# abiswas-odu/Disco

Hardware: AMD Instinct MI355X
Metric: overlaps/sec (BuildGraph stage), 150 bp reads (higher is better)
Workload: dtype u64; 1 GPU; 50000000 x 150 bp synthetic reads, 30x of 50 x 5000000 bp uniform-random contigs, both strands, error-free, min-overlap 40 (k=39), transitive reduction on, seed 42; reads=50000000, read_len=150, min_overlap=40, parallelism=1 GPU, e_pre=903537181, e_out=45314794, n_contained=4685156, cap_bind_sites=0, asymmetric_pairs=0, probes=5550000000, kmer_hits=2220071992

## Files before the change

disco_amd/csrc/disco_hip.hip:

```cpp
#include <hip/hip_runtime.h>
#include <rocprofiler-sdk-roctx/roctx.h>

#include <algorithm>
#include <atomic>
#include <chrono>
#include <cstdarg>
#include <cstdio>
#include <cstdlib>
#include <cstring>
#include <functional>
#include <fcntl.h>
#include <sys/mman.h>
#include <sys/stat.h>
#include <unistd.h>
#include <string>
#include <memory>
#include <thread>
#include <map>
#include <mutex>
#include <queue>
#include <vector>

#include "../../include/disco_hip.h"
#include "../../include/disco_hip_test.h"
// ... 796 lines not shown
{
    CHK(ensure(c, c->reads_own, words));
    c->d_reads = c->reads_own;
    CHK(ensure(c, c->len_own, n_len));
    c->d_len = c->len_own;
    return DISCO_OK;
}

static u32 extra_cap(const disco_ctx *c) { return (u32)std::min<u64>(std::min(c->d_extra_node.cap, c->d_extra_key.cap), 0xFFFFFFFFull); }

static int grow_big_lists(disco_ctx *c, u64 need) { return ensure_group(c, need, need, c->d_big_list, c->d_big_cnt); }

static bool own_order_wanted(const disco_ctx *c, u64 nq, int *bits)
{
    const u64 order_min = getenv("DISCO_ORDER_MIN_READS") ? (u64)atoll(getenv("DISCO_ORDER_MIN_READS")) : 4096;
    int b = 16;
    while (b < 27 && (1ull << b) < nq) ++b;
    if (const char *e = getenv("DISCO_ORDER_BITS")) b = std::min(std::max(atoi(e), 12), 26);
    *bits = b;
    return !c->order_external && !getenv("DISCO_NO_ORDER") && nq >= order_min && nq > 0;
}

struct IndexCountPlan {
    u64 lo = 0, hi = 0;
    int lpr = 0, nf = 0;
    u32 *ocnt = nullptr, *oslot = nullptr;
    u64 *oitem = nullptr;
    u32 oidbits = 0;
    u32 oshift = 0;
    u32 osub = 0;
    const u64 *list = nullptr;
};

static bool runs_nf_built(int nf, int m) { return (nf == 7 || nf == 12 || nf == 17 || nf == 22 || nf == 27) && m == RUNS_M; }

static int runs_lpr_for(const disco_ctx *c, int nf, u32 max_len, u64 nloc)
{
    int lpr = 0;
    const int m = view(c).m;
    const bool nf_built = runs_nf_built(nf, m);
    const bool nf_generic = nf >= 2 && nf <= 64 && m > 16 && m <= 31 && !getenv("DISCO_NO_GENERIC_RUNS");
    if ((nf_built || nf_generic) && max_len > (u32)c->ks && !getenv("DISCO_NO_RUNS")) {
        const u32 maxwin = max_len - (u32)c->ks;
        const u32 expect = 2u * maxwin / (u32)(nf + 1);
        lpr = maxwin <= 256 ? (maxwin <= 128 && expect <= 20 ? 16 : (expect <= 44 ? 32 : 0)) : 0;
        const double max_gb = getenv("DISCO_RUNS_MAX_GB") ? atof(getenv("DISCO_RUNS_MAX_GB")) : 16.0;
        if ((double)nloc * lpr * 4.0 > max_gb * 1e9) lpr = 0;
    }
    return lpr;
}

static bool two_class_ok(const disco_ctx *c, int S, u64 n, u64 n_long, u32 short_max, bool will_own = false)
{
    if (((c->comm || c->dist_reads) && !c->dist_two_class) || !(c->reads_owned || will_own) || c->prm.max_substitutions || getenv("DISCO_NO_TWO_CLASS")) return false;
    if (S <= VERIFY_SW || n_long == 0 || n_long * (u64)env_int("DISCO_TWO_CLASS_ONE_IN", 5) > n || n + n_long >= (1ull << 31)) return false;
    return runs_lpr_for(c, c->ks - view(c).m + 1, short_max, n) != 0;
}

static int two_class_alloc(disco_ctx *c, u64 n_long, int Sx, u32 short_max)
{
    c->n_long = n_long;
    c->S_ext = Sx;
    int rc = ensure(c, c->d_ovf, c->n_alloc);
    if (rc == DISCO_OK) rc = ensure(c, c->d_full, n_long * (u64)Sx);
    if (rc == DISCO_OK) rc = ensure(c, c->d_long_ids, n_long);
    if (rc == DISCO_OK) rc = ensure(c, c->d_lpos, n_long);
    if (rc == DISCO_OK) rc = ensure(c, c->d_lmeta, n_long);
    if (rc == DISCO_OK) rc = ensure(c, c->d_linfo, n_long);
    if (rc == DISCO_OK) rc = ensure(c, c->d_n_list, 1);
    if (rc != DISCO_OK) {
        free_long_class(c);
        return rc;
    }
    c->S = VERIFY_SW;
    c->tailb = short_max <= 160 ? 160 : 256;
    c->two_class = true;
    if (getenv("DISCO_VERBOSE"))
        fprintf(stderr, "[disco] two classes of rows: %llu of %llu reads are longer than 256 bases, the others up to %u: 64-byte rows + %d-word rows for those\n",
                (unsigned long long)n_long, (unsigned long long)c->n, short_max, Sx);
    return DISCO_OK;
}

static bool binned_order_wanted(disco_ctx *c, u64 n, int obits, int *id_bits)
{
    if (getenv("DISCO_NO_BINNED_ORDER") || getenv("DISCO_NO_ORDERED_FILL") || c->two_class || n != c->n || n >= 0xFFFF0000ull) return false;
    const u64 binned_min = getenv("DISCO_BINNED_ORDER_MIN_READS") ? (u64)atoll(getenv("DISCO_BINNED_ORDER_MIN_READS")) : (1ull << 21);
    if (n < binned_min) return false;
    int idb = 1, lenb = 1;
    while ((1ull << idb) < n) ++idb;
    while ((1u << lenb) <= c->max_len) ++lenb;
    if (obits + lenb + idb > 64) return false;
    if (ensure(c, c->d_rec2, n) != DISCO_OK) {
        (void)hipGetLastError();
        c->err.clear();
        return false;
    }
    *id_bits = idb;
    c->order_spare_bits = 64 - (obits + lenb + idb);
    return true;
}

static int index_count_plan(disco_ctx *c, const DiscoView &v, u64 lo, u64 hi, IndexCountPlan *pl, const u64 *list = nullptr)
{
    const u64 nloc = hi - lo;
    *pl = IndexCountPlan();
    pl->lo = lo;
    pl->hi = hi;
    pl->list = list;
    if (!list) c->order_counted = c->order_ready = c->order_items = false;
    int obits = 0;
    if (!list && lo == c->q_lo && hi == c->q_hi && own_order_wanted(c, nloc, &obits) && !getenv("DISCO_NO_ORDER_FUSE")) {
        const u64 order_buckets = 1ull << obits;
        if (lo == 0 && binned_order_wanted(c, nloc, obits, &c->order_id_bits)) {
            pl->oitem = (u64 *)c->d_rec2.p;
            pl->oidbits = (u32)c->order_id_bits;
            c->order_items = true;
        } else {
            CHK(ensure(c, c->d_ocnt, order_buckets + 1));
            CHK(ensure(c, c->d_oslot, nloc));
            HIPCHK(c, hipMemsetAsync(c->d_ocnt, 0, (order_buckets + 1) * sizeof(u32), c->stream));
            pl->ocnt = c->d_ocnt;
            pl->oslot = c->d_oslot;
        }
        pl->oshift = 32u - (u32)obits;
        c->order_counted = true;
        c->order_counted_lo = lo;
        c->order_counted_hi = hi;
        c->order_counted_bits = obits;
    }
    c->runs_lpr = 0;
    c->runs_n = 0;
    c->runs_by_pos = false;
    const int nf = v.ks - v.m + 1;
    const int lpr = c->S == VERIFY_SW ? runs_lpr_for(c, nf, c->max_len, nloc) : 0;
    if (lpr && nloc) {
        CHK(ensure(c, c->d_runs, nloc * (u64)lpr));
        c->runs_lpr = lpr;
        c->runs_lo = lo;
        c->runs_n = nloc;
        c->runs_by_pos = list != nullptr;
        pl->lpr = lpr;
        pl->nf = nf;
    }
    c->order_sub_bits = 0;
    if (pl->oitem && pl->lpr) {
        const int qbits = std::max(0, std::min(c->order_spare_bits, std::min(c->order_sub_limit, ORDER_SUB_MAX)));
        const u32 nmm_max = c->max_len - (u32)v.m + 1u;
        if (qbits) pl->osub = ((u32)qbits << 24) | ((1u << (qbits + 16)) / nmm_max);
        c->order_sub_bits = qbits;
    }
    return DISCO_OK;
}

typedef void (*IndexRunsFn)(DiscoView, u32 *, ulonglong2 *, u32 *, u64, u64, u32 *, u32 *, u32 *, u64 *, u32, u32, u32, const u64 *);
typedef void (*IndexCountFn)(DiscoView, u32 *, ulonglong2 *, u32 *, u64, u64, u32 *, u32 *, u64 *, u32, u32, const u64 *);
struct IndexCountKernel {
    IndexRunsFn runs = nullptr;
    IndexCountFn plain = nullptr;
};
template <bool COUNT, int NF, int NFMAX, bool LONGK>
static IndexCountKernel index_runs_pick(int lpr)
{
    IndexCountKernel k;
    k.runs = lpr == 16 ? index_runs_kernel<COUNT, NF, 1, NFMAX, LONGK> : index_runs_kernel<COUNT, NF, 2, NFMAX, LONGK>;
    return k;
}
template <bool COUNT>
static IndexCountKernel index_count_pick(int nf, int m, int lpr, bool longk, bool long_class)
{
    if (long_class || !lpr) {
        IndexCountKernel k;
        if (long_class) k.plain = longk ? index_count_kernel<COUNT, true, true> : index_count_kernel<COUNT, false, true>;
        else k.plain = longk ? index_count_kernel<COUNT, true> : index_count_kernel<COUNT>;
        return k;
    }
    if (runs_nf_built(nf, m)) switch (nf) {
        case 7: return index_runs_pick<COUNT, 7, 7, false>(lpr);
        case 12: return index_runs_pick<COUNT, 12, 12, false>(lpr);
        case 17: return index_runs_pick<COUNT, 17, 17, false>(lpr);
        case 22: return index_runs_pick<COUNT, 22, 22, false>(lpr);
        default: return index_runs_pick<COUNT, 27, 27, false>(lpr);
        }
    if (longk) return nf <= 48 ? index_runs_pick<COUNT, 0, 48, true>(lpr) : index_runs_pick<COUNT, 0, 64, true>(lpr);
    if (nf <= 8) return index_runs_pick<COUNT, 0, 8, false>(lpr);
    if (nf <= 12) return index_runs_pick<COUNT, 0, 12, false>(lpr);
    if (nf <= 16) return index_runs_pick<COUNT, 0, 16, false>(lpr);
    if (nf <= 24) return index_runs_pick<COUNT, 0, 24, false>(lpr);
    if (nf <= 32) return index_runs_pick<COUNT, 0, 32, false>(lpr);
    if (nf <= 48) return index_runs_pick<COUNT, 0, 48, false>(lpr);
    return index_runs_pick<COUNT, 0, 64, false>(lpr);
}
static IndexCountKernel index_count_pick(bool count, int nf, int m, int lpr, bool longk, bool long_class)
{
    return count ? index_count_pick<true>(nf, m, lpr, longk, long_class) : index_count_pick<false>(nf, m, lpr, longk, long_class);
}

static int index_count_chunk(disco_ctx *c, const DiscoView &v, const IndexCountPlan &pl, bool count, ulonglong2 *rec_base, u64 a, u64 b)
{
    if (b <= a) return DISCO_OK;
    const dim3 grid((unsigned)((b - a + 255) / 256));
    ulonglong2 *rec = rec_base + 2 * (a - pl.lo);
    u32 *oslot = pl.oslot ? pl.oslot + (a - pl.lo) : nullptr;
    u64 *oitem = pl.oitem ? pl.oitem + (a - pl.lo) : nullptr;
    u32 *okey = pl.list ? nullptr : c->d_okey.p;
    const IndexCountKernel k = index_count_pick(count, pl.nf, v.m, pl.lpr, c->ks > 64, false);
    if (k.runs) hipLaunchKernelGGL(k.runs, grid, dim3(256), 0, c->stream, v, c->d_bkt, rec, okey, a, b, c->d_runs + (a - pl.lo) * (u64)pl.lpr, pl.ocnt, oslot, oitem, pl.oidbits, pl.oshift, pl.osub, pl.list);
    else hipLaunchKernelGGL(k.plain, grid, dim3(256), 0, c->stream, v, c->d_bkt, rec, okey, a, b, pl.ocnt, oslot, oitem, pl.oidbits, pl.oshift, pl.list);
    HIPCHK(c, hipGetLastError());
    return DISCO_OK;
}

static int index_count_long(disco_ctx *c, const DiscoView &v, const IndexCountPlan &pl, bool count, ulonglong2 *rec, u32 *oslot, u64 x_lo, u64 x_hi)
{
    const dim3 g((unsigned)((x_hi - x_lo + 255) / 256));
    hipLaunchKernelGGL(index_count_pick(count, 0, v.m, 0, c->ks > 64, true).plain, g, dim3(256), 0, c->stream, v, c->d_bkt, rec, c->d_okey, x_lo, x_hi, pl.ocnt, oslot, (u64 *)nullptr, 0u, pl.oshift,
                       (const u64 *)nullptr);
    HIPCHK(c, hipGetLastError());
    return DISCO_OK;
}

static bool binned_index_wanted(disco_ctx *c, int logT)
{
    if (getenv("DISCO_NO_BINNED_INDEX") || 2 * c->n >= 0xFFFF0000ull) return false;
    if (logT > BINX_SPAN_BITS && ensure(c, c->d_rec2, 2 * c->n) != DISCO_OK) {
        (void)hipGetLastError();
        c->err.clear();
        return false;
    }
    return true;
}

static int size_bucket_table(disco_ctx *c)
{
    u64 T = 1024;
    int logT = 10;
    double tscale = 2.0;
    if (const char *e = getenv("DISCO_BUCKET_SCALE")) tscale = atof(e);
    while ((double)T < tscale * (double)c->n && logT < 32) {
        T <<= 1;
        logT++;
    }
    c->T = T;
    c->bshift = 64 - logT;
    return logT;
}

static int index_begin(disco_ctx *c)
{
    const int logT = size_bucket_table(c);
    const u64 T = c->T;
    CHK(ensure(c, c->d_bkt, T + 1));
    CHK(ensure(c, c->d_ent, 2 * c->n));
    CHK(ensure(c, c->d_rec, 2 * c->n));
    CHK(ensure(c, c->d_okey, c->n));
    c->adj_imported = false;
    c->binned_index = binned_index_wanted(c, logT);
    if (!c->binned_index) HIPCHK(c, hipMemsetAsync(c->d_bkt, 0, (T + 1) * sizeof(u32), c->stream));
    return DISCO_OK;
}

struct BinxPlan {
    int span = 0, levels = 0, bits[3] = {0, 0, 0};
};
static BinxPlan binx_plan(int logT)
{
    BinxPlan b;
    b.span = std::min(logT, BINX_SPAN_BITS);
    const int prefix = logT - b.span;
    b.levels = (prefix + BINX_MAX_BITS - 1) / BINX_MAX_BITS;
    for (int l = 0; l < b.levels; l++) b.bits[l] = prefix / b.levels + (l < prefix % b.levels ? 1 : 0);
    return b;
}

template <typename R>
static int binx_partition(disco_ctx *c, const char *what, int bits, u32 kshift, u32 total, R *src, R *dst, const R **out, const u32 **part)
{
    const BinxPlan bp = binx_plan(bits);
    const u32 n_part = 1u << (bits - bp.span);
    const u32 tiles = (total + BINX_TILE - 1u) / BINX_TILE;
    u64 hist_len = 1;
    for (int l = 0, done = 0; l < bp.levels; done += bp.bits[l], l++) hist_len = std::max<u64>(hist_len, ((u64)tiles + (1ull << done)) * (1ull << bp.bits[l]) + 1);
    const u64 tab = ((u64)n_part + 1 + 63) & ~63ull;
    CHK(ensure(c, c->d_binx, 4 * tab + hist_len));
    u32 *seg[2] = {c->d_binx.p, c->d_binx.p + tab}, *tb[2] = {c->d_binx.p + 2 * tab, c->d_binx.p + 3 * tab}, *hist = c->d_binx.p + 4 * tab;
    if (getenv("DISCO_VERBOSE"))
        fprintf(stderr, "[disco] binned %s: 2^%d buckets, %u partitions of 2^%d, %d level(s) of %d / %d / %d bits\n", what, bits, n_part, bp.span, bp.levels, bp.bits[0], bp.bits[1], bp.bits[2]);
    u32 pseg = 1, pnb = 1;
    int cur = 0, done = 0;
    for (int l = 0; l < bp.levels; l++) {
        const u32 nseg = 1u << done, nb = 1u << bp.bits[l], shift = kshift + (u32)(bits - done - bp.bits[l]);
        const u32 grid = tiles + nseg;
        const u64 hlen = (u64)grid * nb + 1;
        hipLaunchKernelGGL(binx_segs_kernel, dim3(1), dim3(1024), 0, c->stream, l ? (const u32 *)hist : (const u32 *)nullptr, (const u32 *)tb[cur ^ 1], pseg, pnb, total, seg[cur], tb[cur]);
        HIPCHK(c, hipMemsetAsync(hist, 0, hlen * sizeof(u32), c->stream));
        hipLaunchKernelGGL(binx_hist_kernel<R>, dim3(grid), dim3(BINX_BLOCK), 0, c->stream, (const R *)src, (const u32 *)seg[cur], (const u32 *)tb[cur], nseg, shift, nb, hist);
        CHK((scan_exclusive<u32, u32>(c, hist, hlen, hist, false, nullptr)));
        hipLaunchKernelGGL(binx_scatter_kernel<R>, dim3(grid), dim3(BINX_BLOCK), 0, c->stream, (const R *)src, dst, (const u32 *)seg[cur], (const u32 *)tb[cur], nseg, shift, nb, (const u32 *)hist);
        HIPCHK(c, hipGetLastError());
        std::swap(src, dst);
        pseg = nseg;
        pnb = nb;
        done += bp.bits[l];
        cur ^= 1;
    }
    hipLaunchKernelGGL(binx_segs_kernel, dim3(1), dim3(1024), 0, c->stream, bp.levels ? (const u32 *)hist : (const u32 *)nullptr, (const u32 *)tb[cur ^ 1], pseg, pnb, total, seg[cur],
                       (u32 *)nullptr);
    HIPCHK(c, hipGetLastError());
    *out = src;
    *part = seg[cur];
    return DISCO_OK;
}

static int binned_build_index(disco_ctx *c)
{
    const int logT = 64 - c->bshift;
    const u32 total = (u32)(2 * c->n);
    const ulonglong2 *rec;
    const u32 *part;
    CHK(binx_partition(c, "index build", logT, 32u, total, c->d_rec.p, c->d_rec2.p, &rec, &part));
    const int span = std::min(logT, BINX_SPAN_BITS);
    hipLaunchKernelGGL(binx_build_kernel<ulonglong2>, dim3(1u << (logT - span)), dim3(BINX_BUILD_BLOCK), 0, c->stream, rec, part, (u32)span, 32u, 0u, total, c->T, c->d_bkt.p, c->d_ent.p);
    HIPCHK(c, hipGetLastError());
    return DISCO_OK;
}

static int binned_build_order(disco_ctx *c)
{
    const int bits = c->order_counted_bits + c->order_sub_bits;
    const u32 total = (u32)c->n, kshift = 64u - (u32)bits;
    u64 *items = (u64 *)c->d_rec2.p;
    const u64 *rec;
    const u32 *part;
    CHK(binx_partition(c, "grouping", bits, kshift, total, items, items + c->n, &rec, &part));
    const int span = std::min(bits, BINX_SPAN_BITS);
    hipLaunchKernelGGL(binx_build_kernel<u64>, dim3(1u << (bits - span)), dim3(BINX_BUILD_BLOCK), 0, c->stream, rec, part, (u32)span, kshift, (u32)c->order_id_bits, total, (u64)0,
                       (u32 *)nullptr, c->d_order_own.p);
    HIPCHK(c, hipGetLastError());
    return DISCO_OK;
}

static int start_contained_rows(disco_ctx *c, bool grouped)
{
    const u64 nc = c->n_contained;
    if (c->crows_pending && c->crows_n == nc && (!grouped || c->cgrp_pending)) return DISCO_OK;
    const bool have_rows = c->crows_pending && c->crows_n == nc;
    if (!have_rows) c->crows_pending = c->cgrp_pending = false;
    const u64 max_rows = getenv("DISCO_EAGER_ROWS_MAX") ? (u64)atoll(getenv("DISCO_EAGER_ROWS_MAX")) : (16ull << 20);
    if (c->comm || nc == 0 || nc > max_rows || c->n >= (1ull << 31)) return DISCO_OK;
    if (!c->aux_stream) {
        HIPCHK(c, hipStreamCreateWithFlags(&c->aux_stream, hipStreamNonBlocking));
        HIPCHK(c, hipEventCreateWithFlags(&c->ev_crows, hipEventDisableTiming));
        HIPCHK(c, hipMalloc((void **)&c->d_total2, sizeof(u64)));
    }
    CHK(ensure(c, c->d_cpos, c->n + 1));
    CHK(ensure_group(c, nc, nc + nc / 4 + 1024, c->d_crow_id, c->d_crow_key, c->d_crow_len));
    if (nc > c->crows_hcap && c->h_ring && !c->crows_in_ring && (u64)c->ring_half * 2 >= (nc + 1024) * 32) {
        if (c->h_crows) (void)hipHostFree(c->h_crows);
        c->h_crows = c->h_ring;
        c->crows_hcap = (u64)c->ring_half * 2 / 32;
        c->crows_in_ring = true;
    }
    if (nc > c->crows_hcap) {
        if (c->h_crows && !c->crows_in_ring) (void)hipHostFree(c->h_crows);
        c->crows_in_ring = false;
        c->h_crows = nullptr;
        c->crows_hcap = 0;
        const u64 want = nc + nc / 4 + 1024;
        if (hipHostMalloc(&c->h_crows, want * 32) != hipSuccess) {
            c->h_crows = nullptr;
            (void)hipGetLastError();
            return DISCO_OK;
        }
        c->crows_hcap = want;
    }
    if (!have_rows) {
    CHK((scan_exclusive_on<u8, u32>(c, c->aux_stream, c->d_tile2, c->d_total2, c->d_contained, c->n, c->d_cpos, false, nullptr)));
    hipLaunchKernelGGL(contain_rows32_kernel, dim3(flat_grid(c, c->n)), dim3(256), 0, c->aux_stream, c->d_best, c->d_contained, c->d_cpos, c->n, c->d_crow_id, c->d_crow_key);
    HIPCHK(c, hipGetLastError());
    u64 *hkey = (u64 *)c->h_crows;
    u32 *hid = (u32 *)(hkey + c->crows_hcap), *hln = hid + c->crows_hcap;
    hipLaunchKernelGGL(crow_lens_kernel, dim3(flat_grid(c, nc)), dim3(256), 0, c->aux_stream, (const u32 *)c->d_crow_id, (const u64 *)c->d_crow_key, nc, (const u16 *)c->d_len, c->d_crow_len);
    HIPCHK(c, hipGetLastError());
    HIPCHK(c, hipMemcpyAsync(hkey, c->d_crow_key, nc * 8, hipMemcpyDeviceToHost, c->aux_stream));
    HIPCHK(c, hipMemcpyAsync(hid, c->d_crow_id, nc * 4, hipMemcpyDeviceToHost, c->aux_stream));
    HIPCHK(c, hipMemcpyAsync(hln, c->d_crow_len, nc * 4, hipMemcpyDeviceToHost, c->aux_stream));
    HIPCHK(c, hipEventRecord(c->ev_crows, c->aux_stream));
    c->crows_n = nc;
    c->crows_pending = true;
    }
    if (grouped && !c->cgrp_pending) {
        CHK(ensure(c, c->d_cgrp_cur, c->n + 1));
        CHK(ensure_group(c, nc, nc + nc / 4 + 1024, c->d_cgrp_id, c->d_cgrp_key));
        CHK(ensure(c, c->d_cgrp_big, 1));
        HIPCHK(c, hipMemsetAsync(c->d_cpos, 0, (c->n + 1) * sizeof(u32), c->aux_stream));
        HIPCHK(c, hipMemsetAsync(c->d_cgrp_big, 0, sizeof(u64), c->aux_stream));
        hipLaunchKernelGGL(crow_count_kernel, dim3(flat_grid(c, nc)), dim3(256), 0, c->aux_stream, (const u64 *)c->d_crow_key, nc, c->d_cpos);
        CHK((scan_exclusive_on<u32, u32>(c, c->aux_stream, c->d_tile2, c->d_total2, c->d_cpos, c->n + 1, c->d_cgrp_cur, false, nullptr)));
        hipLaunchKernelGGL(crow_place_kernel, dim3(flat_grid(c, nc)), dim3(256), 0, c->aux_stream, (const u32 *)c->d_crow_id, (const u64 *)c->d_crow_key, nc, c->d_cgrp_cur, c->d_cgrp_id,
                           c->d_cgrp_key);
        hipLaunchKernelGGL(crow_sort_groups_kernel, dim3(flat_grid(c, nc)), dim3(256), 0, c->aux_stream, c->d_cgrp_id, c->d_cgrp_key, nc, c->d_cgrp_big);
        HIPCHK(c, hipGetLastError());
        u64 *gkey = (u64 *)((char *)c->h_crows + c->crows_hcap * 16);
        u32 *gid = (u32 *)(gkey + c->crows_hcap), *gln = gid + c->crows_hcap;
        hipLaunchKernelGGL(crow_lens_kernel, dim3(flat_grid(c, nc)), dim3(256), 0, c->aux_stream, (const u32 *)c->d_cgrp_id, (const u64 *)c->d_cgrp_key, nc, (const u16 *)c->d_len, c->d_crow_len);
        HIPCHK(c, hipMemcpyAsync(gkey, c->d_cgrp_key, nc * 8, hipMemcpyDeviceToHost, c->aux_stream));
        HIPCHK(c, hipMemcpyAsync(gid, c->d_cgrp_id, nc * 4, hipMemcpyDeviceToHost, c->aux_stream));
        HIPCHK(c, hipMemcpyAsync(gln, c->d_crow_len, nc * 4, hipMemcpyDeviceToHost, c->aux_stream));
        HIPCHK(c, hipMemcpyAsync(&c->h_cgrp_big, c->d_cgrp_big, sizeof(u64), hipMemcpyDeviceToHost, c->aux_stream));
        c->cgrp_pending = true;
    }
    return DISCO_OK;
}

static int settle_contained_rows(disco_ctx *c)
{
    if (c->crows_pending) HIPCHK(c, hipStreamSynchronize(c->aux_stream));
    c->crows_pending = false;
    c->cgrp_pending = false;
    return DISCO_OK;
}

static int ring_back_from_rows(disco_ctx *c)
{
    if (!c->crows_in_ring) return DISCO_OK;
    if (c->crows_pending && c->aux_stream) HIPCHK(c, hipStreamSynchronize(c->aux_stream));
    c->crows_pending = c->cgrp_pending = false;
    c->h_crows = nullptr;
    c->crows_hcap = 0;
    c->crows_in_ring = false;
    return DISCO_OK;
}

static void settle_hits_prealloc(disco_ctx *c)
{
    if (!c->hits_prealloc.joinable()) return;
    c->hits_prealloc.join();
    c->hbm_bytes -= std::exchange(c->prealloc_asked, 0) * 8;
    if (c->prealloc && c->prealloc.cap > c->d_hits.cap) {
        release(c, c->d_hits);
        adopt(c, c->d_hits, c->prealloc);
    } else if (c->prealloc)
        (void)hipFree(c->prealloc.p);
    c->prealloc = DevBuf<u64>();
}


typedef void (*ProbeFn)(ProbeArgs);
typedef void (*ProbeRunsFn)(ProbeArgs, const u32 *, u64);
struct ProbeKernel {
    ProbeRunsFn runs = nullptr;
    ProbeFn plain = nullptr;
};
template <int PMODE>
static ProbeFn probe_mode_pick(bool ldsrow, bool row17, bool longk, bool long_class)
{
    if constexpr (PMODE != 0) {
        if (long_class) return longk ? probe_kernel<PMODE, false, false, true, true> : row17 ? probe_kernel<PMODE, false, true, false, true> : probe_kernel<PMODE, false, false, false, true>;
    }
    if constexpr (PMODE != 2) {
        if (!ldsrow) return longk ? probe_kernel<PMODE, false, false, true> : row17 ? probe_kernel<PMODE, false, true> : probe_kernel<PMODE, false, false>;
    }
    return longk ? probe_kernel<PMODE, true, false, true> : row17 ? probe_kernel<PMODE, true, true> : probe_kernel<PMODE, true, false>;
}
static ProbeKernel probe_pick(const disco_ctx *c, int mode, bool use_runs)
{
    const bool ldsrow = c->S <= PROBE_ACAP;
    const bool row17 = c->ks - view(c).m == 16 && !getenv("DISCO_NO_ROW17");
    const bool longk = c->ks > 64;
    const bool long_class = c->two_class && c->S_ext > PROBE_ACAP;
    ProbeKernel k;
    if (mode == 0 && use_runs) k.runs = c->k != c->ks ? (c->runs_lpr == 16 ? probe_runs_kernel<16, true> : probe_runs_kernel<32, true>) : (c->runs_lpr == 16 ? probe_runs_kernel<16> : probe_runs_kernel<32>);
    else if (mode == 0) k.plain = probe_mode_pick<0>(ldsrow, row17, longk, long_class);
    else if (mode == 1) k.plain = probe_mode_pick<1>(ldsrow, row17, longk, long_class);
    else k.plain = probe_mode_pick<2>(ldsrow, row17, longk, long_class);
    return k;
}

typedef void (*VerifyFn)(VerifyArgs);
template <bool INEXACT>
static VerifyFn verify_rows_pick(int S, bool short_rows)
{
    if (S == VERIFY_SW) return short_rows ? verify_kernel<5, 0, INEXACT> : verify_kernel<8, 0, INEXACT>;
    return S == 16 ? verify_kernel<16, 0, INEXACT> : S == 24 ? verify_kernel<24, 0, INEXACT> : S == 32 ? verify_kernel<32, 0, INEXACT> : verify_kernel<0, 0, INEXACT>;
}
template <int MODE>
static VerifyFn verify_pass_pick(bool flat, bool short_rows)
{
    if (flat) return short_rows ? verify_flat_kernel<5, MODE> : verify_flat_kernel<8, MODE>;
// ... 341 lines not shown
        return fail(c, DISCO_E_ARG, "%llu reads have a length outside (min_overlap=%u, min(32767, 32*stride)]", (unsigned long long)c->h_ctr[CTR_BAD_LEN], c->prm.min_overlap);
    c->max_len = (u32)c->h_ctr[CTR_MAX_LEN];
    c->phase = 1;
    return DISCO_OK;
}

struct ReadShape {
    u64 n = 0;
    uint32_t stride = 0;
    u64 n_long = 0;
    u32 short_max = 0, longest = 0, shortest = 0;
};

static void set_read_lengths(disco_ctx *c, u32 longest, u32 short_max, u32 shortest)
{
    c->max_len_all = longest;
    c->max_len = c->two_class ? short_max : longest;
    c->min_len = shortest;
}

static void drop_reads(disco_ctx *c) { (void)set_reads_common(c, 0, VERIFY_SW, nullptr); }

static int begin_rows(disco_ctx *c, u64 n, u64 n_alloc, u64 extra_rows, uint32_t stride, bool may_keep, bool spare_hits = false)
{
    LocalBuf<u64> hits(c);
    bool kept = false;
    if (spare_hits) hits.take(c->d_hits);
    const int rc = set_reads_common(c, n, stride, may_keep ? &kept : nullptr);
    if (spare_hits) hits.give(c->d_hits);
    CHK(rc);
    c->reads_owned = true;
    c->n_alloc = n_alloc;
    return kept ? DISCO_OK : alloc_reads(c, (n_alloc + extra_rows) * (u64)stride, n_alloc);
}

static int begin_read_table(disco_ctx *c, const ReadShape &s, bool spare_hits = false)
{
    const bool classes = two_class_ok(c, (int)s.stride, s.n, s.n_long, s.short_max, true);
    CHK(begin_rows(c, s.n, s.n, classes ? s.n_long : 0, classes ? (uint32_t)VERIFY_SW : s.stride, !classes, spare_hits));
    if (classes) CHK(two_class_alloc(c, s.n_long, (int)s.stride, s.short_max));
    set_read_lengths(c, s.longest, s.short_max, s.shortest);
    return DISCO_OK;
}

static int number_long_reads(disco_ctx *c, u32 *ovf, u32 *ids, u64 *count)
{
    hipLaunchKernelGGL(class_flag_kernel, dim3(flat_grid(c, c->n)), dim3(256), 0, c->stream, (const u16 *)c->d_len, c->n, ovf, c->d_ctr);
    CHK((scan_exclusive<u32, u32>(c, ovf, c->n, ovf, false, count)));
    if (ids) hipLaunchKernelGGL(class_ids_kernel, dim3(flat_grid(c, c->n)), dim3(256), 0, c->stream, (const u16 *)c->d_len, (const u32 *)ovf, c->n, ids);
    return DISCO_OK;
}

static int upload_reads_impl(disco_ctx *c, const char *who, const uint64_t *packed, uint32_t stride_words, const uint16_t *len, uint64_t n)
{
    if (!c || (n && (!packed || !len))) return c ? fail(c, DISCO_E_ARG, "%s: null argument", who) : DISCO_E_ARG;
    HIPCHK(c, hipSetDevice(c->device));
    const bool ragged = stride_words == 0;
    const auto t_begin = std::chrono::steady_clock::now();
    auto lapms = [&]() { return std::chrono::duration<double, std::milli>(std::chrono::steady_clock::now() - t_begin).count(); };
    double t_scan = 0, t_alloc = 0, t_issued = 0, t_mirror = 0;
    u64 CH = getenv("DISCO_UPLOAD_CHUNK") ? (u64)atoll(getenv("DISCO_UPLOAD_CHUNK")) : (4ull << 20);
    if (!ragged) CH = std::min<u64>(CH, (512ull << 20) / ((u64)stride_words * 8));
    CH = std::max<u64>((CH + 255) & ~255ull, 256);
    const u64 n_chunks = (n + CH - 1) / CH;
    u64 n_bad = 0;
    ReadShape shape{n, 0, 0, 0, 0, n ? 0xFFFFu : 0u};
    std::vector<u64> chunk_words(n_chunks + 1, 0);
    {
        const u32 mo = c->prm.min_overlap, cap = ragged ? 32767u : std::min<u32>(32767u, stride_words * 32u);
        std::mutex mu;
        parallel_for(n, [&](u64 b0, u64 e0) {
            u64 bad = 0, nlong = 0;
            u32 mx = 0, mn = 0xFFFFu, smx = 0;
            for (u64 k = b0 / CH; k * CH < e0; k++) {
                u64 words = 0;
                for (u64 i = std::max<u64>(b0, k * CH); i < std::min<u64>(e0, (k + 1) * CH); i++) {
                    const u32 L = len[i];
                    bad += (L <= mo || L > cap);
                    mx = std::max(mx, L);
                    mn = std::min(mn, L);
                    nlong += L > (u32)DISCO_SHORT_MAX;
                    if (L <= (u32)DISCO_SHORT_MAX) smx = std::max(smx, L);
                    words += (L + 31u) >> 5;
                }
                std::lock_guard<std::mutex> lk(mu);
                chunk_words[k + 1] += words;
            }
            std::lock_guard<std::mutex> lk(mu);
            n_bad += bad;
            shape.n_long += nlong;
            shape.longest = std::max(shape.longest, mx);
            shape.shortest = std::min(shape.shortest, mn);
            shape.short_max = std::max(shape.short_max, smx);
        });
        for (u64 k = 0; k < n_chunks; k++) chunk_words[k + 1] += chunk_words[k];
    }
    if (ragged) stride_words = std::max<u32>(1, (shape.longest + 31) / 32);
    t_scan = lapms();
    const uint32_t dstride = shape.stride = (stride_words + 7u) & ~7u;
    if (n_bad) {
        drop_reads(c);
        return fail(c, DISCO_E_ARG, "%llu reads have a length outside (min_overlap=%u, min(32767, 32*stride)]", (unsigned long long)n_bad, c->prm.min_overlap);
    }
    CHK(begin_read_table(c, shape));
    const bool classes = c->two_class;
    if (n) {
        CHK(ensure_copy_stream(c));
        CHK(copy_stream_after_stream(c));
        const bool direct = !ragged && !classes && dstride == stride_words;
        const bool eager = !c->comm && !classes && !getenv("DISCO_NO_EAGER_INDEX");
        HIPCHK(c, hipMemcpyAsync(c->d_len, len, n * 2, hipMemcpyHostToDevice, c->stream));
        u64 ring_words = 0;
        for (u64 k = 0; k < n_chunks; k++)
            ring_words = std::max<u64>(ring_words, ragged ? chunk_words[k + 1] - chunk_words[k] : (std::min<u64>(n, (k + 1) * CH) - k * CH) * (u64)stride_words);
        if (!direct) CHK(ensure(c, c->d_dense, 3 * ring_words));
        LocalBuf<u64> woff(c);
        LocalBuf<u32> nw(c);
        if (ragged) {
            CHK(ensure(c, woff, n));
            CHK(ensure(c, nw, n));
            hipLaunchKernelGGL(words_per_read_kernel, dim3(flat_grid(c, n)), dim3(256), 0, c->stream, (const u16 *)c->d_len, n, nw);
            CHK((scan_exclusive<u32, u64>(c, nw, n, woff, false, nullptr)));
        }
        if (classes) CHK(number_long_reads(c, c->d_ovf, c->d_long_ids, nullptr));
        t_alloc = lapms();
        IndexCountPlan pl;
        DiscoView v;
        if (eager) {
            CHK(index_begin(c));
            v = view(c);
            CHK(index_count_plan(c, v, 0, n, &pl));
        }
        for (u64 k = 0; k < n_chunks; k++) {
            const u64 lo = k * CH, hi = std::min<u64>(n, lo + CH);
            const int b = (int)(k % 3);
            if (!direct) {
                u64 *ring = c->d_dense + (u64)b * ring_words;
                const u64 w0 = ragged ? chunk_words[k] : lo * (u64)stride_words, w1 = ragged ? chunk_words[k + 1] : hi * (u64)stride_words;
                if (k >= 3) HIPCHK(c, hipStreamWaitEvent(c->copy_stream, c->ev_unpacked[b], 0));
                HIPCHK(c, hipMemcpyAsync(ring, packed + w0, (w1 - w0) * 8, hipMemcpyHostToDevice, c->copy_stream));
                HIPCHK(c, hipEventRecord(c->ev_copied[b], c->copy_stream));
                HIPCHK(c, hipStreamWaitEvent(c->stream, c->ev_copied[b], 0));
                hipLaunchKernelGGL(unpack_reads_kernel, dim3(flat_grid(c, (hi - lo) * (u64)c->S)), dim3(256), 0, c->stream, (const u64 *)ring, ragged ? 0 : (int)stride_words, (const u64 *)woff, w0,
                                   (const u16 *)c->d_len, lo, hi, c->S, classes ? (u32)DISCO_SHORT_MAX : 0xFFFFu, c->d_reads);
                if (classes)
                    hipLaunchKernelGGL(unpack_long_reads_kernel, dim3(flat_grid(c, shape.n_long * ((u64)dstride + 8))), dim3(256), 0, c->stream, (const u64 *)ring, ragged ? 0 : (int)stride_words,
                                       (const u64 *)woff, w0, (const u16 *)c->d_len, lo, hi, (const u32 *)c->d_long_ids, shape.n_long, n, (int)dstride, c->tailb, c->d_full, c->d_reads);
                HIPCHK(c, hipEventRecord(c->ev_unpacked[b], c->stream));
            } else {
                HIPCHK(c, hipMemcpyAsync(c->d_reads + lo * dstride, packed + lo * dstride, (hi - lo) * (u64)dstride * 8, hipMemcpyHostToDevice, c->copy_stream));
                HIPCHK(c, hipEventRecord(c->ev_copied[b], c->copy_stream));
                HIPCHK(c, hipStreamWaitEvent(c->stream, c->ev_copied[b], 0));
            }
            if (eager) CHK(index_count_chunk(c, v, pl, !c->binned_index, c->d_rec, lo, hi));
        }
        HIPCHK(c, hipGetLastError());
        t_issued = lapms();
        if (c->h_len.size() != n) c->h_len.resize(n);
        uint16_t *hl = c->h_len.data();
        parallel_for(n, [&, hl](u64 b0, u64 e0) { memcpy(hl + b0, len + b0, (e0 - b0) * 2); });
        c->h_len_ok = true;
        t_mirror = lapms();
        HIPCHK(c, hipStreamSynchronize(c->copy_stream));
        if (getenv("DISCO_VERBOSE"))
            fprintf(stderr, "[disco] %s: lengths checked %.1f ms, buffers %.1f, chunks issued %.1f, lengths mirrored %.1f, copies done %.1f (%s%s)\n", who, t_scan, t_alloc, t_issued,
                    t_mirror, lapms(), classes ? "two classes of rows" : "one stride", eager ? ", index counted behind the copies" : "");
        if (woff) HIPCHK(c, hipStreamSynchronize(c->stream));
        c->index_counted = eager;
    } else
        c->h_len.clear();
    c->phase = 1;
    return DISCO_OK;
}

int disco_upload_reads(disco_ctx *c, const uint64_t *packed, uint32_t stride_words, const uint16_t *len, uint64_t n)
{
    DISCO_TRACE("disco_upload_reads");
    if (c && stride_words == 0) return fail(c, DISCO_E_ARG, "stride_words 0 out of range");
    return upload_reads_impl(c, "disco_upload_reads", packed, stride_words, len, n);
}

int disco_upload_reads_ragged(disco_ctx *c, const uint64_t *words, const uint16_t *len, uint64_t n)
{
    DISCO_TRACE("disco_upload_reads_ragged");
    return upload_reads_impl(c, "disco_upload_reads_ragged", words, 0, len, n);
}

namespace {
enum { DP_STARTS = 0, DP_GOOD, DP_TOO_LONG, DP_MAX_LEN, DP_MIN_LEN_INV, DP_N_LONG, DP_SHORT_MAX, DP_COUNT };

struct IngestPiece {
    u64 p0 = 0, p1 = 0;
    u64 own_lo = 0, own_hi = 0, n = 0;
    bool to_eof = false;
    bool prefix_nl = true, last_nl = false;
    u64 own_nl = 0, tiles = 0;
    u8 *d_text = nullptr;
    u64 *d_tile_base = nullptr, *d_ctr = nullptr;
    u32 *d_tile_cnt = nullptr;
    u64 *d_start = nullptr, *d_seq = nullptr;
    u32 *d_wrap = nullptr;
    u16 *d_glen = nullptr;
    u64 n_start = 0, good = 0;
    u64 fig[DP_COUNT] = {0, 0, 0, 0, 0, 0, 0};
};

struct IngestFile {
    std::string path;
    int fd = -1;
    char last = 0;
    bool fastq = false;
    u64 n = 0;
    const u8 *map = nullptr;
    u64 comp_n = 0;
    u8 *d_comp = nullptr;
    std::vector<infl::BgzfBlock> blocks;
    uint64_t m_first = 0, m_count = 0;
    IngestPiece p;
};
}

static void ingest_tables(FxTables *tb)
{
    memset(tb, 0, sizeof *tb);
    auto code = [](char ch) { return ch == 'A' ? 0ull : (ch == 'C' ? 1ull : (ch == 'G' ? 2ull : 3ull)); };
    tb->n_rep = (u32)DISCO_N_END_REPEATS;
    for (u32 r = 0; r < tb->n_rep; r++) {
        u64 v = 0;
        for (int x = 0; x < 29; x++) v = (v << 2) | code(kEndRepeats[r][x]);
        tb->rep58[r] = v;
    }
    tb->n_motif = (u32)DISCO_N_MOTIFS;
    for (u32 m = 0; m < tb->n_motif; m++) {
        const size_t l = strlen(kMotifs[m]);
        tb->motif_len[m] = (u8)l;
        for (size_t x = 0; x < l; x++) {
            tb->motif[m][x] = (u8)kMotifs[m][x];
            tb->need[m][code(kMotifs[m][x])]++;
        }
    }
    static_assert(DISCO_N_END_REPEATS <= FX_MAX_REPEATS && DISCO_N_MOTIFS <= FX_MAX_MOTIFS, "filter tables");
}

static unsigned ring_alloc_flags()
{
    const int mode = env_int("DISCO_RING_MODE", 0);
    return mode == 1 ? hipHostMallocNonCoherent : (mode == 2 ? hipHostMallocCoherent : hipHostMallocDefault);
}

static const size_t RING_HALF = 128u << 20;
static int pinned_ring(disco_ctx *c, const char *who)
{
    CHK(ring_back_from_rows(c));
    if (!c->h_ring) {
        if (hipHostMalloc(&c->h_ring, 2 * RING_HALF, ring_alloc_flags()) != hipSuccess) {
            c->h_ring = nullptr;
            (void)hipGetLastError();
            return fail(c, DISCO_E_NOMEM, "%s: no pinned staging memory", who);
        }
        c->ring_half = RING_HALF;
        for (int i = 0; i < 2; i++) HIPCHK(c, hipEventCreateWithFlags(&c->ev_ring[i], hipEventDisableTiming));
    }
    return DISCO_OK;
}
static int ingest_ring(disco_ctx *c)
{
    CHK(pinned_ring(c, "disco_ingest_fasta"));
    return ensure_copy_stream(c);
}

static int ingest_read_file(disco_ctx *c, int fd, u64 n, u8 *d_text, unsigned threads, u64 file_off = 0, void *own_ring = nullptr, size_t own_ring_bytes = 0)
{
    constexpr unsigned RING_SLOTS = 4;
    const size_t HALF = 128u << 20, SLOT = own_ring ? own_ring_bytes / RING_SLOTS : 2 * HALF / RING_SLOTS;
    if (own_ring) CHK(ensure_copy_stream(c));
    else CHK(ingest_ring(c));
    char *const h_ring = own_ring ? (char *)own_ring : (char *)c->h_ring;
    hipEvent_t ev[RING_SLOTS] = {own_ring ? c->ev_copied[2] : c->ev_ring[0], own_ring ? c->ev_unpacked[1] : c->ev_ring[1], c->ev_copied[0], c->ev_copied[1]};
    threads = (unsigned)env_int("DISCO_INGEST_THREADS", (int)std::min(threads, 6u));
    threads = std::max(1u, std::min(threads, 64u));
    CHK(copy_stream_after_stream(c));
    const u64 n_chunks = (n + SLOT - 1) / SLOT;
    const u64 n_pieces = n_chunks * threads;
    std::atomic<u64> next_piece{0};
    std::vector<std::atomic<int>> slot_free(n_chunks), pieces_in(n_chunks);
    for (u64 k = 0; k < n_chunks; k++) {
        slot_free[k].store(k < RING_SLOTS ? 1 : 0);
        pieces_in[k].store(0);
    }
    std::atomic<bool> ok{true}, stop{false};
    auto nap = [] { std::this_thread::sleep_for(std::chrono::microseconds(30)); };
    std::vector<std::thread> th;
    for (unsigned t = 0; t < threads; t++)
        th.emplace_back([&]() {
            for (;;) {
                const u64 p = next_piece.fetch_add(1);
                if (p >= n_pieces) return;
                const u64 k = p / threads;
                const unsigned piece = (unsigned)(p % threads);
                while (!slot_free[k].load(std::memory_order_acquire)) {
                    if (stop.load()) return;
                    nap();
                }
                const u64 off = k * (u64)SLOT;
                const size_t len = (size_t)std::min<u64>(SLOT, n - off);
                char *slot = h_ring + (k % RING_SLOTS) * SLOT;
                size_t p0 = len * piece / threads, p1 = len * (piece + 1) / threads;
// ... 610 lines not shown
            });
    }
    return DISCO_OK;
}

extern "C" int disco_ingest_fetch(disco_ctx *c, uint16_t *len, uint64_t *file_index)
{
    if (!c || !len || !file_index) return c ? fail(c, DISCO_E_ARG, "disco_ingest_fetch: null argument") : DISCO_E_ARG;
    if (c->phase < 1 || c->ingest_n == 0 || c->ingest_n != c->n) return fail(c, DISCO_E_STATE, "disco_ingest_fetch: the reads of the context did not come from disco_ingest_fasta");
    HIPCHK(c, hipSetDevice(c->device));
    const u64 n = c->n;
    CHK(ingest_fetch_range(c, 0, n, c->copy_stream ? c->copy_stream : c->stream, len, file_index));
    {
        std::lock_guard<std::mutex> lk(c->h_len_mu);
        if (!(c->h_len_ok && c->h_len.size() == n)) {
            if (c->h_len.size() != n) c->h_len.resize(n);
            uint16_t *hl = c->h_len.data();
            parallel_for(n, [&, hl](u64 b, u64 e_) { memcpy(hl + b, len + b, (e_ - b) * 2); });
            c->h_len_ok = true;
        }
    }
    return DISCO_OK;
}

int disco_adopt_reads(disco_ctx *c, const void *d_packed, uint32_t stride_words, const void *d_len, uint64_t n)
{
    if (!c || (n && (!d_packed || !d_len))) return c ? fail(c, DISCO_E_ARG, "disco_adopt_reads: null argument") : DISCO_E_ARG;
    HIPCHK(c, hipSetDevice(c->device));
    CHK(set_reads_common(c, n, stride_words));
    c->d_reads = (u64 *)d_packed;
    c->d_len = (u16 *)d_len;
    c->reads_owned = false;
    return validate_reads(c);
}

static int gen_spec(disco_ctx *c, const char *who, const disco_genspec_abi *s, disco_genspec *g, uint32_t *stride)
{
    memcpy(g, s, sizeof *g);
    const uint32_t longest = std::max<uint32_t>(s->len_max, DISCO_GEN_LONG_SHARE(g) ? DISCO_GEN_LONG_LEN(g) : 0u);
    if (s->len_min == 0 || s->len_max < s->len_min || longest > 32767 || s->n_contigs == 0 || s->contig_len < longest) return fail(c, DISCO_E_ARG, "%s: bad spec", who);
    *stride = (((longest + 31) / 32) + 7u) & ~7u;
    return DISCO_OK;
}

int disco_generate_reads(disco_ctx *c, const disco_genspec_abi *s)
{
    DISCO_TRACE("disco_generate_reads");
    if (!c || !s) return c ? fail(c, DISCO_E_ARG, "disco_generate_reads: null argument") : DISCO_E_ARG;
    disco_genspec g;
    ReadShape shape;
    CHK(gen_spec(c, "disco_generate_reads", s, &g, &shape.stride));
    HIPCHK(c, hipSetDevice(c->device));
    shape.n = s->n_reads;
    CHK(begin_read_table(c, shape));
    if (c->n) hipLaunchKernelGGL(generate_reads_kernel, dim3(flat_grid(c, c->n * shape.stride)), dim3(256), 0, c->stream, g, c->d_reads, c->d_len, (int)shape.stride, (u64)0, c->n);
    HIPCHK(c, hipGetLastError());
    return validate_reads(c);
}

int disco_substitute_bases(disco_ctx *c, uint64_t seed, uint32_t rate_ppm)
{
    if (!c) return DISCO_E_ARG;
    if (c->phase != 1) return fail(c, DISCO_E_STATE, "disco_substitute_bases: call after the reads are set and before disco_build_index");
    if (rate_ppm > 1000000) return fail(c, DISCO_E_ARG, "disco_substitute_bases: rate above 10^6 ppm");
    if (c->two_class)
        return fail(c, DISCO_E_UNSUPPORTED, "disco_substitute_bases: the table has two classes of rows (reads of more than 256 bases next to short ones); substitute "
                                            "into generated reads, or set DISCO_NO_TWO_CLASS=1");
    HIPCHK(c, hipSetDevice(c->device));
    const u64 lo = c->comm ? c->q_lo : 0, hi = c->comm ? c->q_hi : c->n;
    if (hi > lo && rate_ppm)
        hipLaunchKernelGGL(substitute_bases_kernel, dim3(flat_grid(c, (hi - lo) * (u64)c->S)), dim3(256), 0, c->stream, (u64)seed, rate_ppm, c->d_reads, c->d_len, c->S, lo, hi);
    c->index_counted = c->order_counted = c->order_ready = false;
    HIPCHK(c, hipGetLastError());
    return DISCO_OK;
}

int disco_download_reads(disco_ctx *c, uint64_t *packed, uint16_t *len)
{
    if (!c || c->phase < 1) return c ? fail(c, DISCO_E_STATE, "no reads") : DISCO_E_ARG;
    HIPCHK(c, hipSetDevice(c->device));
    LocalBuf<u64> joined(c);
    if (packed && c->n && c->two_class) {
        CHK(ensure(c, joined, c->n * (u64)c->S_ext));
        hipLaunchKernelGGL(class_join_kernel, dim3(flat_grid(c, c->n * (u64)c->S_ext)), dim3(256), 0, c->stream, (const u64 *)c->d_reads, (const u64 *)c->d_full, c->S_ext,
                           (const u16 *)c->d_len, (const u32 *)c->d_ovf, c->n, joined);
        (void)hipMemcpyAsync(packed, joined, c->n * (u64)c->S_ext * 8, hipMemcpyDeviceToHost, c->stream);
    } else if (packed && c->n)
        HIPCHK(c, hipMemcpyAsync(packed, c->d_reads, c->n * (u64)c->S * 8, hipMemcpyDeviceToHost, c->stream));
    if (len && c->n) (void)hipMemcpyAsync(len, c->d_len, c->n * 2, hipMemcpyDeviceToHost, c->stream);
    const hipError_t e = hipStreamSynchronize(c->stream);
    if (e != hipSuccess) return fail(c, DISCO_E_HIP, "disco_download_reads: %s", hipGetErrorString(e));
    return DISCO_OK;
}

uint32_t disco_stride_words(const disco_ctx *c) { return c ? (uint32_t)(c->two_class ? c->S_ext : c->S) : 0; }
uint64_t disco_num_reads(const disco_ctx *c) { return c ? c->n : 0; }
uint64_t disco_long_rows(const disco_ctx *c) { return c && c->two_class ? c->n_long : 0; }

int disco_set_query_range(disco_ctx *c, uint64_t lo, uint64_t hi)
{
    if (!c) return DISCO_E_ARG;
    if (c->phase < 1 || c->phase > 2) return fail(c, DISCO_E_STATE, "disco_set_query_range: call after the reads are set and before disco_probe");
    if (lo > hi || hi > c->n) return fail(c, DISCO_E_ARG, "query range [%llu,%llu) outside [0,%llu)", (unsigned long long)lo, (unsigned long long)hi, (unsigned long long)c->n);
    c->q_lo = lo;
    c->q_hi = hi;
    return DISCO_OK;
}

static int two_class_convert(disco_ctx *c)
{
    if (c->two_class || !c->n || c->max_len <= (u32)DISCO_SHORT_MAX || !two_class_ok(c, c->S, c->n, 1, (u32)c->k + 1)) return DISCO_OK;
    const int Sx = c->S;
    LocalBuf<u32> ovf(c);
    CHK(ensure(c, ovf, c->n_alloc));
    CHK(zero_counter(c, CTR_SHORT_MAX));
    u64 n_long = 0;
    CHK(number_long_reads(c, ovf, nullptr, &n_long));
    CHK(read_counters(c));
    const u32 short_max = (u32)c->h_ctr[CTR_SHORT_MAX];
    if (!two_class_ok(c, Sx, c->n, n_long, short_max)) return DISCO_OK;
    LocalBuf<u64> rows8(c);
    ovf.give(c->d_ovf);
    int rca = ensure(c, rows8, (c->n + n_long) * 8);
    if (rca == DISCO_OK) rca = two_class_alloc(c, n_long, Sx, short_max);
    if (rca != DISCO_OK) {
        free_long_class(c);
        return rca;
    }
    hipLaunchKernelGGL(class_split_kernel, dim3(flat_grid(c, c->n * 8)), dim3(256), 0, c->stream, (const u64 *)c->reads_own, Sx, (const u16 *)c->d_len, (const u32 *)c->d_ovf, c->n, c->tailb,
                       rows8.p, c->d_full, c->d_long_ids);
    HIPCHK(c, hipGetLastError());
    HIPCHK(c, hipStreamSynchronize(c->stream));
    rows8.give(c->reads_own);
    c->d_reads = c->reads_own;
    set_read_lengths(c, c->max_len, short_max, c->min_len);
    return DISCO_OK;
}

int disco_build_index(disco_ctx *c)
{
    DISCO_TRACE("disco_build_index");
    if (!c) return DISCO_E_ARG;
    if (c->phase < 1) return fail(c, DISCO_E_STATE, "disco_build_index: no reads");
    HIPCHK(c, hipSetDevice(c->device));
    ph_begin(c, DISCO_PH_INDEX);
    if (c->index_counted) {
        c->index_counted = false;
    } else {
        CHK(two_class_convert(c));
        CHK(index_begin(c));
        const DiscoView v = view(c);
        IndexCountPlan pl;
        CHK(index_count_plan(c, v, 0, c->n, &pl));
        CHK(index_count_chunk(c, v, pl, !c->binned_index, c->d_rec, 0, c->n));
        if (c->two_class) CHK(index_count_long(c, v, pl, !c->binned_index, c->d_rec, pl.oslot, 0, c->n_long));
    }
    const bool binned = c->binned_index;
    if (!binned) CHK((scan_exclusive<u32, u32>(c, c->d_bkt, c->T + 1, c->d_bkt, false, nullptr)));
    c->order_ready = false;
    if (c->order_counted && c->order_counted_lo == 0 && c->order_counted_hi == c->n && !c->two_class && !getenv("DISCO_NO_ORDERED_FILL")) {
        const u64 order_buckets = 1ull << c->order_counted_bits;
        CHK(ensure(c, c->d_order_own, c->n));
        ph_end(c, DISCO_PH_INDEX);
        ph_begin(c, DISCO_PH_ORDER);
        if (c->order_items) CHK(binned_build_order(c));
        else {
            CHK((scan_exclusive<u32, u32>(c, c->d_ocnt, order_buckets + 1, c->d_ocnt, false, nullptr)));
            hipLaunchKernelGGL(order_scatter_kernel, dim3(flat_grid(c, c->n)), dim3(256), 0, c->stream, c->d_okey, c->d_oslot, c->d_ocnt, 32u - (u32)c->order_counted_bits, (u64)0, c->n, c->d_len, c->d_order_own);
        }
        ph_end(c, DISCO_PH_ORDER);
        ph_begin(c, DISCO_PH_INDEX2);
        if (binned) CHK(binned_build_index(c));
        else hipLaunchKernelGGL(index_fill_ordered_kernel, dim3(flat_grid(c, c->n)), dim3(256), 0, c->stream, c->n, (const u64 *)c->d_order_own, (const ulonglong2 *)c->d_rec, (const u32 *)c->d_bkt, c->d_ent);
        ph_end(c, DISCO_PH_INDEX2);
        HIPCHK(c, hipGetLastError());
        c->order_ready = true;
        c->phase = 2;
        return DISCO_OK;
    }
    if (binned) CHK(binned_build_index(c));
    else if (c->n) hipLaunchKernelGGL(index_fill_kernel, dim3(flat_grid(c, 2 * c->n)), dim3(256), 0, c->stream, 2 * c->n, c->d_rec, c->d_bkt, c->d_ent);
    HIPCHK(c, hipGetLastError());
    ph_end(c, DISCO_PH_INDEX);
    c->phase = 2;
    return DISCO_OK;
}

int disco_probe(disco_ctx *c)
{
    DISCO_TRACE("disco_probe");
    if (!c) return DISCO_E_ARG;
    if (c->phase < 2) return fail(c, DISCO_E_STATE, "disco_probe: build the index first");
    HIPCHK(c, hipSetDevice(c->device));
    CHK(settle_contained_rows(c));
    CHK(settle_keys(c));
    drop_edge_records(c);
    drop_contained_records(c);
    settle_hits_prealloc(c);
    const u64 nq = c->q_hi - c->q_lo;
    CHK(ensure(c, c->d_best, c->n_alloc));
    CHK(ensure(c, c->d_row_start, c->n));
    CHK(ensure(c, c->d_row_cnt, c->n));
    if (c->n_alloc) hipLaunchKernelGGL(fill_u64_kernel, dim3(flat_grid(c, c->n_alloc)), dim3(256), 0, c->stream, c->d_best, c->n_alloc, DISCO_NOKEY);
    HIPCHK(c, hipMemsetAsync(c->d_row_cnt, 0, std::max<u64>(c->n, 1) * sizeof(u32), c->stream));
    const bool use_runs = c->runs_lpr != 0 && c->d_runs && c->q_lo >= c->runs_lo && c->q_hi <= c->runs_lo + c->runs_n;
    const ProbeKernel range_kernel = probe_pick(c, 0, use_runs);
    const int grid = range_kernel.runs ? wq_grid(c, range_kernel.runs, nq, "DISCO_PROBE_WAVES") : wq_grid(c, range_kernel.plain, nq, "DISCO_PROBE_WAVES");
    auto launch_probe = [&](const ProbeArgs &a, const ProbeKernel &k, int g) {
        if (k.runs) hipLaunchKernelGGL(k.runs, dim3(g), dim3(64), 0, c->stream, a, (const u32 *)c->d_runs, c->runs_by_pos ? ~0ull : c->runs_lo);
        else hipLaunchKernelGGL(k.plain, dim3(g), dim3(64), 0, c->stream, a);
    };
    const u64 chunk_slots = use_runs ? PR_CHUNK : PROBE_CHUNK;
    u64 want_hits = nq * 64 + (u64)grid * chunk_slots + (1u << 16);
    u32 want_slow = use_runs ? (u32)std::min<u64>(nq, nq / 64 + 1024 + (c->two_class ? c->n_long : 0)) : 1u;
    u32 want_big = (u32)std::min<u64>(nq, nq / 64 + 1024);
    for (int attempt = 0; attempt < 8; attempt++) {
        if (want_hits > c->d_hits.cap) {
            release(c, c->d_hits);
            size_t fr = 0, tot = 0;
            HIPCHK(c, hipMemGetInfo(&fr, &tot));
            if (want_hits * 8 > fr) {
                u64 can = fr / 8 / 10 * 9;
                if (can < (u64)grid * chunk_slots * 2) return fail(c, DISCO_E_NOMEM, "disco_probe: not enough HBM for the hit buffer (%llu entries wanted)", (unsigned long long)want_hits);
                want_hits = can;
            }
            CHK(ensure(c, c->d_hits, want_hits));
        }
        if (want_slow > c->d_slow_list.cap) CHK(ensure(c, c->d_slow_list, want_slow));
        CHK(grow_big_lists(c, want_big));
        HIPCHK(c, hipMemsetAsync(c->d_bump, 0, sizeof(u64), c->stream));
        HIPCHK(c, hipMemsetAsync(c->d_n_big, 0, sizeof(u32), c->stream));
        HIPCHK(c, hipMemsetAsync(c->d_n_slow, 0, sizeof(u32), c->stream));
        HIPCHK(c, hipMemsetAsync(c->d_ctr + CTR_KMER_HITS, 0, sizeof(u64) * 4, c->stream));
        CHK(zero_counter(c, CTR_MAX_ROW));
        CHK(zero_counter(c, CTR_ES_BIG));
        CHK(zero_counter(c, CTR_ES_MID));
        c->es_big_counted = c->tr_big_counted = false;
        ProbeArgs a;
        a.v = view(c);
        a.hits = c->d_hits;
        a.row_start = c->d_row_start;
        a.row_cnt = c->d_row_cnt;
        c->h_probe_rare.bump = c->d_bump;
        c->h_probe_rare.hits_cap = c->d_hits.cap;
        c->h_probe_rare.big_list = c->d_big_list;
        c->h_probe_rare.big_cnt = c->d_big_cnt;
        c->h_probe_rare.n_big = c->d_n_big;
        c->h_probe_rare.big_cap = c->d_big_list.cap;
        c->h_probe_rare.slow_cap = c->d_slow_list.cap;
        c->h_probe_rare.slow_list = c->d_slow_list;
        c->h_probe_rare.n_slow = c->d_n_slow;
        c->h_probe_rare.ctr = c->d_ctr;
        CHK(ensure(c, c->d_probe_rare, 1));
        HIPCHK(c, hipMemcpyAsync(c->d_probe_rare, &c->h_probe_rare, sizeof(ProbeRare), hipMemcpyHostToDevice, c->stream));
        a.rare = c->d_probe_rare;
        CHK(ensure(c, c->d_meta_ord, std::max<u64>(nq, 1)));
        a.meta_ord = c->d_meta_ord;
        int order_bits = 16;
        const bool own_order = own_order_wanted(c, nq, &order_bits);
        a.order = nullptr;
        const u64 order_buckets = 1ull << order_bits;
        const bool counted = c->order_counted && c->order_counted_lo == c->q_lo && c->order_counted_hi == c->q_hi && c->order_counted_bits == order_bits &&
                             (!c->order_items || c->order_ready);
        c->order_counted = false;
        if (c->loci) {
            c->d_order_used = c->d_order_own;
        } else if (own_order && c->order_ready && counted) {
            c->d_order_used = c->d_order_own;
        } else if (own_order) {
            CHK(ensure(c, c->d_ocnt, order_buckets + 1));
            CHK(ensure(c, c->d_oslot, nq));
            CHK(ensure(c, c->d_order_own, nq));
            const u32 oshift = 32u - (u32)order_bits;
            ph_begin(c, DISCO_PH_ORDER);
            if (!counted) {
                HIPCHK(c, hipMemsetAsync(c->d_ocnt, 0, (order_buckets + 1) * sizeof(u32), c->stream));
                hipLaunchKernelGGL(order_count_kernel, dim3(flat_grid(c, nq)), dim3(256), 0, c->stream, c->d_okey + c->q_lo, nq, oshift, c->d_ocnt, c->d_oslot);
            }
            CHK((scan_exclusive<u32, u32>(c, c->d_ocnt, order_buckets + 1, c->d_ocnt, false, nullptr)));
            hipLaunchKernelGGL(order_scatter_kernel, dim3(flat_grid(c, nq)), dim3(256), 0, c->stream, c->d_okey + c->q_lo, c->d_oslot, c->d_ocnt, oshift, c->q_lo, nq, c->d_len, c->d_order_own);
            ph_end(c, DISCO_PH_ORDER);
            HIPCHK(c, hipGetLastError());
            c->d_order_used = c->d_order_own;
        } else if (c->order_external && nq) {
            CHK(ensure(c, c->d_order_own, nq));
            hipLaunchKernelGGL(order_pack_kernel, dim3(flat_grid(c, nq)), dim3(256), 0, c->stream, c->d_order, nq, c->d_len, c->d_order_own);
            HIPCHK(c, hipGetLastError());
            c->d_order_used = c->d_order_own;
        } else
            c->d_order_used = nullptr;
        a.order = c->d_order_used;
        c->order_q_lo = c->q_lo;
        c->order_q_hi = c->q_hi;
        ph_begin(c, DISCO_PH_PROBE_KERNEL);
        HIPCHK(c, hipMemsetAsync(c->d_wq, 0, sizeof(u64) * WQ_WORDS, c->stream));
        const bool partitioned = c->dist_active && c->part_index;
        if (partitioned) CHK(dist_partitioned_probe(c));
        else if (nq) {
            launch_probe(a, range_kernel, grid);
        }
        ph_end(c, DISCO_PH_PROBE_KERNEL);
        HIPCHK(c, hipGetLastError());
        u32 n_big = 0, n_slow = 0;
        if (!partitioned) {
            HIPCHK(c, hipMemcpyAsync(&n_slow, c->d_n_slow, sizeof(u32), hipMemcpyDeviceToHost, c->stream));
            HIPCHK(c, hipMemcpyAsync(&n_big, c->d_n_big, sizeof(u32), hipMemcpyDeviceToHost, c->stream));
        }
        CHK(read_counters(c));
// ... 2404 lines not shown
        sc[(size_t)p] = scnt[(size_t)p] * elem;
        a += sc[(size_t)p];
        ro[(size_t)p] = b;
        rc[(size_t)p] = rcnt[(size_t)p] * elem;
        b += rc[(size_t)p];
        if (p != c->comm->rank) c->dinfo.bytes_sent[xid] += sc[(size_t)p];
    }
    const auto t0 = HClock::now();
    COMM_CHK(c, c->comm->all_to_all_v(send, so.data(), sc.data(), recv, ro.data(), rc.data(), c->stream));
    if (c->time_exchanges) HIPCHK(c, hipStreamSynchronize(c->stream));
    c->dinfo.ms[xid] += ms_since(t0);
    return DISCO_OK;
}

static u64 vsum(const std::vector<u64> &v)
{
    u64 s = 0;
    for (u64 x : v) s += x;
    return s;
}

static int host_reduce(disco_ctx *c, u64 *vals, int n, bool take_max = false)
{
    const int G = c->comm->world;
    std::vector<u64> all((size_t)G * n);
    COMM_CHK(c, c->comm->host_all_gather((const unsigned long long *)vals, n, (unsigned long long *)all.data(), c->stream));
    for (int i = 0; i < n; i++) {
        u64 a = 0;
        for (int p = 0; p < G; p++) a = take_max ? std::max(a, all[(size_t)p * n + i]) : a + all[(size_t)p * n + i];
        vals[i] = a;
    }
    return DISCO_OK;
}

template <int W>
static int dist_deal_rows(disco_ctx *c)
{
    typedef ReadItem<W> Item;
    const u64 nhome = c->home_hi - c->home_lo;
    const u64 per16 = (sizeof(Item) + 15) / 16;
    CHK(ensure(c, c->d_x16a, std::max<u64>(2 * nhome * per16, 1)));
    Item *items = (Item *)c->d_x16a.p, *sorted = (Item *)(c->d_x16a + nhome * per16);
    if (nhome) hipLaunchKernelGGL(read_items_kernel<W>, dim3(flat_grid(c, nhome * (W + 1))), dim3(256), 0, c->stream, (const u64 *)c->d_reads, (const u16 *)c->d_len, c->S, c->home_lo, c->home_hi, items);
    HIPCHK(c, hipGetLastError());
    std::vector<u64> scnt, rcnt;
    RouteByReadItem<W> f{c->d_otab};
    CHK(route_items(c, items, nhome, f, sorted, scnt));
    CHK(exchange_counts(c, scnt, rcnt));
    const u64 nr = vsum(rcnt);
    if (nr != c->n_own) return fail(c, DISCO_E_STATE, "dealt reads: %llu rows arrive for %llu own reads", (unsigned long long)nr, (unsigned long long)c->n_own);
    CHK(ensure(c, c->d_x16b, std::max<u64>(nr * per16, 1)));
    CHK(a2a_items(c, DISCO_X_READS_DEALT, sorted, scnt, c->d_x16b, rcnt, sizeof(Item)));
    if (nr) hipLaunchKernelGGL(read_items_place_kernel<W>, dim3(flat_grid(c, nr * (W + 1))), dim3(256), 0, c->stream, (const Item *)c->d_x16b.p, nr, c->S, c->d_reads, c->d_len);
    HIPCHK(c, hipGetLastError());
    return DISCO_OK;
}

static int dist_deal_reads(disco_ctx *c)
{
    DISCO_TRACE("dist_deal_reads");
    const u32 G = (u32)c->comm->world, r = (u32)c->comm->rank;
    const u64 hlo = c->home_lo, hhi = c->home_hi;
    CHK(ensure(c, c->d_okey, c->n_alloc));
    CHK(ensure(c, c->d_otab, c->n_alloc));
    DiscoView v = view(c);
    if (hhi > hlo) {
        if (v.m == RUNS_M) hipLaunchKernelGGL(read_keys_kernel<true>, dim3((unsigned)((hhi - hlo + 255) / 256)), dim3(256), 0, c->stream, v, hlo, hhi, c->d_okey);
        else hipLaunchKernelGGL(read_keys_kernel<false>, dim3((unsigned)((hhi - hlo + 255) / 256)), dim3(256), 0, c->stream, v, hlo, hhi, c->d_okey);
    }
    HIPCHK(c, hipGetLastError());
    {
        const auto t0 = HClock::now();
        COMM_CHK(c, c->comm->all_gather(c->d_okey + (u64)r * c->per, c->d_okey, c->per * sizeof(u32), c->stream));
        c->dinfo.bytes_sent[DISCO_X_KEYS] += (u64)(G - 1) * c->per * sizeof(u32);
        c->dinfo.ms[DISCO_X_KEYS] += ms_since(t0);
    }
    CHK(ensure(c, c->d_own_ids, std::max<u64>(c->n, 1)));
    CHK(ensure(c, c->d_list_n, 1));
    HIPCHK(c, hipMemsetAsync(c->d_list_n, 0, sizeof(u64), c->stream));
    int obits = 16;
    const bool order_own = own_order_wanted(c, std::max<u64>(c->n / G, 1), &obits) && !getenv("DISCO_DIST_ORDER_TWO_PASSES");
    const u32 oshift = 32u - (u32)obits;
    if (order_own) {
        CHK(ensure(c, c->d_ocnt, (1ull << obits) + 1));
        CHK(ensure(c, c->d_oslot, std::max<u64>(c->n, 1)));
        HIPCHK(c, hipMemsetAsync(c->d_ocnt, 0, ((1ull << obits) + 1) * sizeof(u32), c->stream));
    }
    if (c->n) hipLaunchKernelGGL(own_select_kernel, dim3((unsigned)std::min<u64>((c->n + OWN_TILE - 1) / OWN_TILE, (u64)c->n_cu * 16)), dim3(256), 0, c->stream, (const u32 *)c->d_okey, c->n, G, r,
                                 c->d_otab, c->d_own_ids, c->d_list_n, order_own ? c->d_ocnt : (u32 *)nullptr, order_own ? c->d_oslot : (u32 *)nullptr, oshift);
    HIPCHK(c, hipGetLastError());
    u64 n_own = 0;
    HIPCHK(c, hipMemcpyAsync(&n_own, c->d_list_n, sizeof(u64), hipMemcpyDeviceToHost, c->stream));
    HIPCHK(c, counted_stream_sync(c->stream));
    c->n_own = n_own;
    c->loci = true;
    c->q_lo = 0;
    c->q_hi = n_own;
    if (c->wait_bulk_before_verify) {
        const int W = (int)((c->max_len + 31) / 32);
        if (W <= 5 && c->S >= 5 && !getenv("DISCO_DIST_NO_DEAL_ROWS")) CHK(dist_deal_rows<5>(c));
        else if (W <= 8 && c->S >= 8 && !getenv("DISCO_DIST_NO_DEAL_ROWS")) CHK(dist_deal_rows<8>(c));
        else {
            HIPCHK(c, hipStreamWaitEvent(c->stream, c->ev_bulk, 0));
            c->wait_bulk_before_verify = false;
        }
    }
    CHK(ensure(c, c->d_order_own, std::max<u64>(n_own, 1)));
    ph_begin(c, DISCO_PH_ORDER);
    int obits2 = 16;
    const bool order_two = !order_own && own_order_wanted(c, n_own, &obits2);
    if ((order_own && n_own) || order_two) {
        const int ob = order_own ? obits : obits2;
        const u64 order_buckets = 1ull << ob;
        const u32 oshift = 32u - (u32)ob;
        if (order_two) {
            CHK(ensure(c, c->d_ocnt, order_buckets + 1));
            CHK(ensure(c, c->d_oslot, n_own));
            HIPCHK(c, hipMemsetAsync(c->d_ocnt, 0, (order_buckets + 1) * sizeof(u32), c->stream));
            hipLaunchKernelGGL(order_count_list_kernel, dim3(flat_grid(c, n_own)), dim3(256), 0, c->stream, (const u32 *)c->d_okey, (const u32 *)c->d_own_ids, n_own, G, r, oshift, c->d_ocnt, c->d_oslot);
        }
        CHK((scan_exclusive<u32, u32>(c, c->d_ocnt, order_buckets + 1, c->d_ocnt, false, nullptr)));
        hipLaunchKernelGGL(order_scatter_list_kernel, dim3(flat_grid(c, n_own)), dim3(256), 0, c->stream, (const u32 *)c->d_okey, (const u32 *)c->d_own_ids, (const u32 *)c->d_oslot,
                           (const u32 *)c->d_ocnt, n_own, G, r, oshift, (const u16 *)c->d_len, c->d_order_own);
    } else if (n_own)
        hipLaunchKernelGGL(order_pack_list_kernel, dim3(flat_grid(c, n_own)), dim3(256), 0, c->stream, (const u32 *)c->d_own_ids, n_own, (const u16 *)c->d_len, c->d_order_own);
    ph_end(c, DISCO_PH_ORDER);
    HIPCHK(c, hipGetLastError());
    c->d_order_used = c->d_order_own;
    c->order_counted = false;
    c->dinfo.own_reads = n_own;
    return DISCO_OK;
}

static int dist_build_index(disco_ctx *c)
{
    DISCO_TRACE("dist_build_index");
    const u32 G = (u32)c->comm->world, r = (u32)c->comm->rank;
    const u64 nloc = c->q_hi - c->q_lo;
    const int logT = size_bucket_table(c);
    const u64 T = c->T;
    auto blo_of = [&](u64 g) { return (g * T + G - 1) / G; };
    const u64 blo = blo_of(r), bhi = blo_of(r + 1);
    const bool part = c->part_index;
    if (!part) {
        CHK(ensure(c, c->d_bkt, T + 1));
        CHK(ensure(c, c->d_ent, 2 * c->n));
    }
    CHK(ensure(c, c->d_okey, c->loci ? c->n_alloc : c->n));
    CHK(ensure(c, c->d_rec, std::max<u64>(2 * nloc, 1)));
    c->adj_imported = false;
    ph_begin(c, DISCO_PH_INDEX);
    DiscoView v = view(c);
    IndexCountPlan pl;
    if (c->loci) {
        CHK(index_count_plan(c, v, 0, c->n_own, &pl, c->d_order_own));
        CHK(index_count_chunk(c, v, pl, false, c->d_rec, 0, c->n_own));
    } else {
        CHK(index_count_plan(c, v, c->q_lo, c->q_hi, &pl));
        CHK(index_count_chunk(c, v, pl, false, c->d_rec, c->q_lo, c->q_hi));
        if (c->two_class && nloc) {
            u32 xb[2] = {0, (u32)c->n_long};
            HIPCHK(c, hipMemcpyAsync(&xb[0], c->d_ovf + c->q_lo, sizeof(u32), hipMemcpyDeviceToHost, c->stream));
            if (c->q_hi < c->n) HIPCHK(c, hipMemcpyAsync(&xb[1], c->d_ovf + c->q_hi, sizeof(u32), hipMemcpyDeviceToHost, c->stream));
            HIPCHK(c, hipStreamSynchronize(c->stream));
            if (xb[1] > xb[0]) {
                ulonglong2 *rec_by_id = c->d_rec - 2 * (ptrdiff_t)c->q_lo;
                u32 *oslot_by_id = pl.oslot ? pl.oslot - (ptrdiff_t)c->q_lo : nullptr;
                CHK(index_count_long(c, v, pl, false, rec_by_id, oslot_by_id, xb[0], xb[1]));
            }
        }
    }
    CHK(ensure(c, c->d_x16a, std::max<u64>(2 * nloc, 1)));
    std::vector<u64> scnt, rcnt, matrix;
    RouteByBucket f{logT, G};
    CHK(route_items(c, c->d_rec.p, 2 * nloc, f, c->d_x16a.p, scnt));
    CHK(exchange_counts(c, scnt, rcnt, &matrix));
    const u64 nrec = vsum(rcnt);
    CHK(ensure(c, c->d_x16b, std::max<u64>(nrec, 1)));
    CHK(a2a_items(c, DISCO_X_INDEX_RECORDS, c->d_x16a, scnt, c->d_x16b, rcnt, sizeof(ulonglong2)));
    std::vector<u64> shard((size_t)G, 0);
    for (u32 p = 0; p < G; p++)
        for (u32 q = 0; q < G; q++) shard[q] += matrix[(size_t)p * G + q];
    u64 base = 0;
    for (u32 q = 0; q < r; q++) base += shard[q];
    if (shard[r] != nrec) return fail(c, DISCO_E_STATE, "index shard: %llu records received, %llu announced", (unsigned long long)nrec, (unsigned long long)shard[r]);
    if (vsum(shard) != 2 * c->n) return fail(c, DISCO_E_STATE, "index: %llu records over all ranks, expected %llu", (unsigned long long)vsum(shard), (unsigned long long)(2 * c->n));
    if (part) {
        CHK(ensure(c, c->d_bkt, bhi - blo + 1));
        CHK(ensure(c, c->d_ent, std::max<u64>(nrec, 1)));
        u32 *bkt0 = c->d_bkt - blo;
        HIPCHK(c, hipMemsetAsync(c->d_bkt, 0, (bhi - blo + 1) * sizeof(u32), c->stream));
        if (nrec) hipLaunchKernelGGL(shard_count_kernel, dim3(flat_grid(c, nrec)), dim3(256), 0, c->stream, c->d_x16b, nrec, bkt0);
        CHK((scan_exclusive<u32, u32>(c, c->d_bkt, bhi - blo + 1, c->d_bkt, false, nullptr)));
        if (nrec) hipLaunchKernelGGL(index_fill_kernel, dim3(flat_grid(c, nrec)), dim3(256), 0, c->stream, nrec, c->d_x16b, bkt0, c->d_ent);
        HIPCHK(c, hipGetLastError());
        c->part_blo = blo;
        c->part_bhi = bhi;
        c->part_nrec = nrec;
        ph_end(c, DISCO_PH_INDEX);
        c->phase = 2;
        return DISCO_OK;
    }
    if (bhi > blo) HIPCHK(c, hipMemsetAsync(c->d_bkt + blo, 0, (bhi - blo) * sizeof(u32), c->stream));
    if (nrec) hipLaunchKernelGGL(shard_count_kernel, dim3(flat_grid(c, nrec)), dim3(256), 0, c->stream, c->d_x16b, nrec, c->d_bkt);
    if (bhi > blo) {
        CHK((scan_exclusive<u32, u32>(c, c->d_bkt + blo, bhi - blo, c->d_bkt + blo, false, nullptr)));
        if (base) hipLaunchKernelGGL(add_u32_kernel, dim3(flat_grid(c, bhi - blo)), dim3(256), 0, c->stream, c->d_bkt + blo, bhi - blo, (u32)base);
    }
    if (nrec) hipLaunchKernelGGL(index_fill_kernel, dim3(flat_grid(c, nrec)), dim3(256), 0, c->stream, nrec, c->d_x16b, c->d_bkt, c->d_ent);
    const u32 total = (u32)(2 * c->n);
    HIPCHK(c, hipMemcpyAsync(c->d_bkt + T, &total, sizeof(u32), hipMemcpyHostToDevice, c->stream));
    HIPCHK(c, hipGetLastError());
    HIPCHK(c, hipStreamSynchronize(c->stream));
    {
        std::vector<size_t> off((size_t)G), cnt((size_t)G);
        const auto t0 = HClock::now();
        for (u32 p = 0; p < G; p++) {
            off[p] = blo_of(p) * sizeof(u32);
            cnt[p] = (blo_of(p + 1) - blo_of(p)) * sizeof(u32);
        }
        c->dinfo.bytes_sent[DISCO_X_INDEX_SHARDS] += (u64)(G - 1) * cnt[r];
        COMM_CHK(c, c->comm->all_gather_v(c->d_bkt + blo, c->d_bkt, off.data(), cnt.data(), c->stream));
        size_t a = 0;
        for (u32 p = 0; p < G; p++) {
            off[p] = a;
            cnt[p] = shard[p] * sizeof(u64);
            a += cnt[p];
        }
        c->dinfo.bytes_sent[DISCO_X_INDEX_SHARDS] += (u64)(G - 1) * cnt[r];
        COMM_CHK(c, c->comm->all_gather_v(c->d_ent + base, c->d_ent, off.data(), cnt.data(), c->stream));
        HIPCHK(c, hipStreamSynchronize(c->stream));
        c->dinfo.ms[DISCO_X_INDEX_SHARDS] += ms_since(t0);
    }
    ph_end(c, DISCO_PH_INDEX);
    c->phase = 2;
    return DISCO_OK;
}

static int dist_partitioned_probe(disco_ctx *c)
{
    DISCO_TRACE("dist_partitioned_probe");
    const u32 G = (u32)c->comm->world, r = (u32)c->comm->rank;
    const u64 lo = c->q_lo, nloc = c->q_hi - c->q_lo;
    DiscoView v = view(c);
    const int nf = v.ks - v.m + 1;
    const bool seeded = c->k != c->ks;
    const bool have_runs = c->runs_lpr != 0 && c->runs_lo == lo && c->runs_n == nloc;
    int logT = 0;
    while ((1ull << logT) < c->T) ++logT;
    CHK(ensure(c, c->d_list_n, 1));
    u32 *d_nslow = c->d_n_slow;
    auto make = [&](ulonglong2 *out, bool collect_slow) {
        const int grid = flat_grid(c, nloc * (u64)c->runs_lpr);
        u32 *slow = collect_slow ? (u32 *)c->d_slow_list.p : nullptr;
        const u32 cap = c->d_slow_list.cap * 2;
        auto fn = seeded ? (c->runs_lpr == 16 ? pq_make_kernel<16, true> : pq_make_kernel<32, true>) : (c->runs_lpr == 16 ? pq_make_kernel<16> : pq_make_kernel<32>);
        hipLaunchKernelGGL(fn, dim3(grid), dim3(256), 0, c->stream, v, (const u32 *)c->d_runs, lo, c->q_hi, r, out, c->d_list_n, slow, cap, d_nslow);
    };
    u64 nq_fast = 0, n_slow = 0;
    const u32 *slow = nullptr;
    if (have_runs) {
        u32 ns = 0;
        for (int attempt = 0;; attempt++) {
            const u32 want = attempt ? ns / 2 + 1024 : (u32)std::min<u64>(nloc, nloc / 128 + 1024);
            if (want > c->d_slow_list.cap) CHK(ensure(c, c->d_slow_list, want));
            HIPCHK(c, hipMemsetAsync(c->d_list_n, 0, sizeof(u64), c->stream));
            HIPCHK(c, hipMemsetAsync(d_nslow, 0, sizeof(u32), c->stream));
            if (nloc) make(nullptr, true);
            HIPCHK(c, hipGetLastError());
            HIPCHK(c, hipMemcpyAsync(&nq_fast, c->d_list_n, sizeof(u64), hipMemcpyDeviceToHost, c->stream));
            HIPCHK(c, hipMemcpyAsync(&ns, d_nslow, sizeof(u32), hipMemcpyDeviceToHost, c->stream));
            HIPCHK(c, hipStreamSynchronize(c->stream));
            if (ns <= c->d_slow_list.cap * 2 || attempt) break;
        }
        if (ns > c->d_slow_list.cap * 2) return fail(c, DISCO_E_CAPACITY, "dist_partitioned_probe: slow list could not be sized");
        n_slow = ns;
        slow = (const u32 *)c->d_slow_list.p;
    } else
        n_slow = nloc;
    u64 nq_slow = 0, nqs = 0;
    {
    LocalBuf<u32> slow_cnt(c);
    LocalBuf<u64> slow_start(c);
    if (n_slow) {
        CHK(ensure(c, slow_cnt, n_slow));
        CHK(ensure(c, slow_start, n_slow + 1));
        if (seeded) hipLaunchKernelGGL((pq_slow_kernel<true, true>), dim3(flat_grid(c, n_slow, 64)), dim3(64), 0, c->stream, v, slow, n_slow, lo, r, slow_cnt, (const u64 *)nullptr, (ulonglong2 *)nullptr);
        else if (c->ks > 64) hipLaunchKernelGGL(pq_slow_kernel<true>, dim3(flat_grid(c, n_slow, 64)), dim3(64), 0, c->stream, v, slow, n_slow, lo, r, slow_cnt, (const u64 *)nullptr, (ulonglong2 *)nullptr);
        else hipLaunchKernelGGL(pq_slow_kernel<false>, dim3(flat_grid(c, n_slow, 64)), dim3(64), 0, c->stream, v, slow, n_slow, lo, r, slow_cnt, (const u64 *)nullptr, (ulonglong2 *)nullptr);
        CHK((scan_exclusive<u32, u64>(c, slow_cnt, n_slow, slow_start, false, &nq_slow)));
    }
    nqs = nq_fast + nq_slow;
    CHK(ensure(c, c->d_x16a, std::max<u64>(2 * nqs, 1)));
    HIPCHK(c, hipMemsetAsync(c->d_list_n, 0, sizeof(u64), c->stream));
    if (have_runs && nloc) make(c->d_x16a, false);
    if (n_slow) {
        if (seeded) hipLaunchKernelGGL((pq_slow_kernel<true, true>), dim3(flat_grid(c, n_slow, 64)), dim3(64), 0, c->stream, v, slow, n_slow, lo, r, slow_cnt, (const u64 *)slow_start, c->d_x16a + nq_fast);
        else if (c->ks > 64) hipLaunchKernelGGL(pq_slow_kernel<true>, dim3(flat_grid(c, n_slow, 64)), dim3(64), 0, c->stream, v, slow, n_slow, lo, r, slow_cnt, (const u64 *)slow_start, c->d_x16a + nq_fast);
        else hipLaunchKernelGGL(pq_slow_kernel<false>, dim3(flat_grid(c, n_slow, 64)), dim3(64), 0, c->stream, v, slow, n_slow, lo, r, slow_cnt, (const u64 *)slow_start, c->d_x16a + nq_fast);
    }
    if (hipGetLastError() != hipSuccess || hipStreamSynchronize(c->stream) != hipSuccess) return fail(c, DISCO_E_HIP, "dist_partitioned_probe: query kernels failed");
    }
    c->slow_rows = have_runs ? n_slow : 0;
    std::vector<u64> scnt, rcnt;
    RouteByBucket fb{logT, G};
    ulonglong2 *q_sorted = c->d_x16a + nqs;
    CHK(route_items(c, c->d_x16a.p, nqs, fb, q_sorted, scnt));
    CHK(exchange_counts(c, scnt, rcnt));
    const u64 nq_in = vsum(rcnt);
    CHK(ensure(c, c->d_x16b, std::max<u64>(nq_in, 1)));
    CHK(a2a_items(c, DISCO_X_QUERIES, q_sorted, scnt, c->d_x16b, rcnt, sizeof(ulonglong2)));
    CHK(ensure(c, c->d_deg_tmp, std::max<u64>(nq_in, 1)));
    CHK(ensure(c, c->d_pq_start, nq_in + 1));
    const u32 *bkt = c->d_bkt;
    u64 n_hits_out = 0;
    auto answer_count = seeded ? pq_answer_kernel<false, true> : pq_answer_kernel<false, false>;
    auto answer_fill = seeded ? pq_answer_kernel<true, true> : pq_answer_kernel<true, false>;
    if (nq_in) hipLaunchKernelGGL(answer_count, dim3(flat_grid(c, nq_in)), dim3(256), 0, c->stream, (const ulonglong2 *)c->d_x16b, nq_in, bkt, (const u64 *)c->d_ent, c->part_blo, c->per,
                                  nf, c->k - c->ks, c->d_deg_tmp, (const u64 *)nullptr, (ulonglong2 *)nullptr);
    CHK((scan_exclusive<u32, u64>(c, c->d_deg_tmp, nq_in, c->d_pq_start, false, &n_hits_out)));
    CHK(ensure_keep(c, c->d_x16a, std::max<u64>(2 * n_hits_out, 1), 0));
// ... 1420 lines not shown
```

disco_amd/csrc/disco_kernels.h:

```cpp
#ifndef DISCO_KERNELS_H_
#define DISCO_KERNELS_H_

#include "disco_device.h"
#include "readgen.h"

#define PROBE_ROWCAP 512
#define PROBE_SEGW 128
#define PROBE_SEGP (PROBE_SEGW + 64)
#define PROBE_ACAP 32
#define PROBE_CHUNK 4096
#define ES_MID 1024
#define ES_DUPBITS 11
#define ES_DUPTAB (1 << ES_DUPBITS)
#ifndef ES_CAP
#define ES_CAP 256
#endif
#ifndef TR_CAP
#define TR_CAP 256
#endif
#define TR_CAP_SMALL 128
#define VERIFY_SW 8
#define ORDER_BUCKET(key, shift) (((key) * 0x9E3779B1u) >> (shift))
#define SCAN_ITEMS 16
#define SCAN_BLOCK 256
// ... 65 lines not shown
template <u32 CHUNK = WQ_CHUNK>
__device__ __forceinline__ bool wq_grab(u64 *counter, u64 n, u64 &beg, u64 &end)
{
    u64 b = 0;
    if ((threadIdx.x & 63) == 0) b = atomicAdd(counter, (u64)CHUNK);
#ifdef WQ_EXP_SHFL
    b = __shfl(b, 0);
#else
    b = uniform_u64(b);
#endif
    beg = b;
    end = (b + CHUNK < n) ? b + CHUNK : n;
    return b < n;
}

template <u32 CHUNK = WQ_CHUNK, u32 MULT = 4>
__device__ __forceinline__ bool wq_grab_multi(u64 *counter, u64 n, u64 &beg, u64 &end, u64 &gnext, u64 &gend)
{
    if (gnext >= gend) {
        if (!wq_grab<CHUNK * MULT>(counter, n, gnext, gend)) return false;
    }
    beg = gnext;
    end = beg + CHUNK < gend ? beg + CHUNK : gend;
    gnext = end;
    return true;
}

#define WQ_NQ 8u
#define WQ_WORDS (16u * WQ_NQ)
struct WqSplit {
    u32 qi = 0;
};
template <u32 CHUNK = WQ_CHUNK>
__device__ __forceinline__ bool wq_grab_split(u64 *counters, u64 n, u64 &beg, u64 &end, WqSplit &st)
{
    const u32 nchunks = (u32)((n + CHUNK - 1u) / CHUNK);
    const u32 per = (nchunks + WQ_NQ - 1u) / WQ_NQ;
    while (st.qi < WQ_NQ) {
        const u32 q = ((u32)blockIdx.x + st.qi) % WQ_NQ;
        const u32 first = q * per;
        const u32 mine = first < nchunks ? (nchunks - first < per ? nchunks - first : per) : 0u;
        u32 b = mine;
        if (mine) {
            u32 t = 0;
            if ((threadIdx.x & 63) == 0) t = atomicAdd((u32 *)&counters[16u * q], 1u);
            b = uniform_u32(t);
        }
        if (b < mine) {
            beg = (u64)(first + b) * CHUNK;
            end = beg + CHUNK < n ? beg + CHUNK : n;
            return true;
        }
        st.qi++;
    }
    return false;
}

struct DiscoView {
    const u64 *reads;
    const u16 *len;
    u64 n;
    int S;
    int k;
    int ks;
    int m;
    const u32 *bkt;
    const u64 *ent;
    int bshift;
    u64 q_lo, q_hi;
    u64 *ctr;
    u64 *wq;
    const u64 *full;
    const u32 *ovf;
    const u32 *long_ids;
    u32 n_long;
    int SL;
    int tailb;
};

struct OwnSet {
    const u8 *otab;
    u32 me;
    u64 lo, hi;
    const u64 *list;
    u64 n_own;
    const u32 *ids;
    __device__ __forceinline__ bool mine(u64 v) const { return otab ? otab[v] == (u8)me : (v >= lo && v < hi); }
    __device__ __forceinline__ u64 count() const { return otab ? n_own : hi - lo; }
    __device__ __forceinline__ u64 node(u64 i) const { return otab ? ORDER_ID(list[i]) : lo + i; }
    __device__ __forceinline__ u64 node_by_id(u64 i) const { return otab ? (u64)ids[i] : lo + i; }
};
__host__ __device__ __forceinline__ u32 disco_key_owner(u32 key, u32 G) { return (u32)(((u64)(key * 0x9E3779B1u) * (u64)G) >> 32); }

__global__ void generate_reads_kernel(disco_genspec spec, u64 *__restrict__ reads, u16 *__restrict__ len, int S, u64 r_lo, u64 r_hi)
{
    u64 gid = r_lo * (u64)S + (u64)blockIdx.x * blockDim.x + threadIdx.x;
    u64 total = r_hi * (u64)S;
    for (; gid < total; gid += (u64)gridDim.x * blockDim.x) {
        u64 r = gid / S;
        int w = (int)(gid % S);
        disco_readloc loc = disco_read_location(&spec, r);
        u64 word = 0;
        int base0 = w * 32;
        for (int i = 0; i < 32; i++) {
            int p = base0 + i;
            if (p < (int)loc.len) word |= (u64)disco_read_base(&spec, &loc, (u32)p) << (62 - 2 * i);
        }
        reads[gid] = word;
        if (w == 0) len[r] = (u16)loc.len;
    }
}

__global__ void substitute_bases_kernel(u64 seed, u32 rate_ppm, u64 *__restrict__ reads, const u16 *__restrict__ len, int S, u64 r_lo, u64 r_hi)
{
    u64 gid = r_lo * (u64)S + (u64)blockIdx.x * blockDim.x + threadIdx.x;
    const u64 total = r_hi * (u64)S;
    for (; gid < total; gid += (u64)gridDim.x * blockDim.x) {
        const u64 r = gid / S;
        const int base0 = (int)(gid % S) * 32, L = (int)len[r];
        if (base0 >= L) continue;
        const u64 word = reads[gid];
        u64 out = 0;
        for (int i = 0; i < 32; i++) {
            u32 b = (u32)(word >> (62 - 2 * i)) & 3u;
            if (base0 + i < L) b = disco_substituted_base(seed, rate_ppm, r, (u32)(base0 + i), b);
            else b = 0;
            out |= (u64)b << (62 - 2 * i);
        }
        reads[gid] = out;
    }
}

__global__ void validate_len_kernel(const u16 *__restrict__ len, u64 n, int S, int min_overlap, u64 *ctr)
{
    u64 i = (u64)blockIdx.x * blockDim.x + threadIdx.x;
    u32 bad = 0, mx = 0, mn = 0xFFFFu;
    for (; i < n; i += (u64)gridDim.x * blockDim.x) {
        u32 L = len[i];
        if (L <= (u32)min_overlap || L > 32767u || L > (u32)S * 32u) bad++;
        mx = L > mx ? L : mx;
        mn = L < mn ? L : mn;
    }
    if (bad) atomicAdd(&ctr[CTR_BAD_LEN], (u64)bad);
    for (int o = 32; o > 0; o >>= 1) {
        mx = max(mx, (u32)__shfl_down(mx, o));
        mn = min(mn, (u32)__shfl_down(mn, o));
    }
    if ((threadIdx.x & 63) == 0) {
        atomicMax(&ctr[CTR_MAX_LEN], (u64)mx);
        atomicMax(&ctr[CTR_MIN_LEN], (u64)(0xFFFFu - mn));
    }
}

template <bool COUNT, bool LONGK = false, bool LONGCLASS = false>
__global__ void __launch_bounds__(256) index_count_kernel(DiscoView v, u32 *__restrict__ bkt, ulonglong2 *__restrict__ rec, u32 *__restrict__ okey, u64 lo, u64 hi,
                                                          u32 *__restrict__ ocnt, u32 *__restrict__ oslot, u64 *__restrict__ oitem, u32 oidbits, u32 oshift,
                                                          const u64 *__restrict__ list = nullptr)
{
    const u64 x = lo + (u64)blockIdx.x * 256u + threadIdx.x;
    if (x >= hi) return;
    const u64 i = LONGCLASS ? (u64)v.long_ids[x] : x;
    const u64 lw = (!LONGCLASS && list) ? list[x] : 0ull;
    const u64 rid = (!LONGCLASS && list) ? ORDER_ID(lw) : i;
    if (LONGCLASS) lo = 0;
    const int S = LONGCLASS ? v.SL : v.S;
    const u64 *__restrict__ p = LONGCLASS ? v.full + x * (u64)S : v.reads + rid * (u64)S;
    if (!LONGCLASS && v.full && v.len[rid] > DISCO_SHORT_MAX) return;
    const int L = (!LONGCLASS && list) ? ORDER_LEN(lw) : (int)v.len[rid], k = v.ks, m = v.m, nf = k - m + 1;
    const int nmm = L - m + 1;
    const int sfx0 = nmm - nf;
    const u64 mask = (1ull << (2 * m)) - 1ull;
    const int rsh = 2 * (m - 1);
    u64 f = 0, r = 0, word = 0;
    int pos = 0;
    auto next = [&]() {
        if ((pos & 31) == 0) word = p[pos >> 5];
        const u32 b = (u32)(word >> 62);
        word <<= 2;
        ++pos;
        f = ((f << 2) | b) & mask;
        r = (r >> 2) | ((u64)(3u - b) << rsh);
    };
    u32 best = 0xFFFFFFFFu;
    auto order_word = [&]() {
        next();
        const bool st = r < f;
        const u32 h = order_hash32(st ? r : f);
        best = min(best, h);
        return (h & ~0x1FFu) | (u32)st;
    };
    for (int q = 0; q < m - 1; ++q) next();
    u32 k1p = 0xFFFFFFFFu, k2p = 0xFFFFFFFFu, k1s = 0xFFFFFFFFu, k2s = 0xFFFFFFFFu;
    int q = 0;
    for (; q < nf; ++q) {
        const u32 o = order_word();
        k1p = min(k1p, o + ((u32)q << 1));
        k2p = min(k2p, o + ((u32)(63 - q) << 1));
        if (q >= sfx0) {
            k1s = min(k1s, o + ((u32)(q - sfx0) << 1));
            k2s = min(k2s, o + ((u32)(63 - (q - sfx0)) << 1));
        }
    }
    for (; q < sfx0; ++q) order_word();
    for (; q < nmm; ++q) {
        const u32 o = order_word();
        k1s = min(k1s, o + ((u32)(q - sfx0) << 1));
        k2s = min(k2s, o + ((u32)(63 - (q - sfx0)) << 1));
    }
    if (okey) okey[i] = best;
    if (oitem) oitem[i - lo] = ORDER_ITEM(best, oshift, rid, L, oidbits);
    else if (ocnt) oslot[i - lo] = atomicAdd(&ocnt[ORDER_BUCKET(best, oshift)], 1u);
    auto resolve = [&](u32 k1, u32 k2, int j0, u32 &t, u32 &rev) {
        const int ffirst = (int)((k1 >> 1) & 63u), flast = 63 - (int)((k2 >> 1) & 63u);
        int fsel = ffirst;
        if (ffirst == flast)
            rev = k1 & 1u;
        else {
            rev = kmer_is_rev<false, LONGK>(p, S, j0, k);
            fsel = rev ? flast : ffirst;
        }
        t = rev ? (u32)(nf - 1 - fsel) : (u32)fsel;
        return mmer_key(p, S, j0 + fsel, m);
    };
    u32 tp, rp, ts, rs;
    const u64 kp = resolve(k1p, k2p, 0, tp, rp);
    const u64 ks = resolve(k1s, k2s, sfx0, ts, rs);
    const u64 bp = kp >> v.bshift, bs = ks >> v.bshift;
    const u32 sp = COUNT ? atomicAdd(&bkt[bp], 1u) : 0u;
    const u32 ss = COUNT ? atomicAdd(&bkt[bs], 1u) : 0u;
    rec[2 * (i - lo)] = make_ulonglong2((bp << 32) | sp, PAY_MAKE(kp, rid, tp, rp, 0, L));
    rec[2 * (i - lo) + 1] = make_ulonglong2((bs << 32) | ss, PAY_MAKE(ks, LONGCLASS ? v.n + x : rid, ts, rs, 1, L));
}

#define RUNS_M 23
template <bool B>
struct FlagConst {
    static constexpr bool value = B;
};
template <int M>
struct MmerRoll {
    static_assert(M == 0 || (M > 16 && M <= 24 && (M & 1)), "two dwords, the high one partly used; a 24-bit fold in order_hash32<false>");
    const u64 *__restrict__ p;
    int last_word;
    u32 himask, rsh;
    int pos = 0;
    u64 word = 0;
    u32 cw = 0;
    u32 flo = 0, fhi = 0, rlo = 0, rhi = 0;
    bool st = false;
    u32 clo = 0, chi = 0;
    __device__ __forceinline__ MmerRoll(const u64 *row, int S, int m = M) : p(row), last_word(S - 1), himask((1u << (2 * m - 32)) - 1u), rsh((u32)(2 * m - 34)) {}
    __device__ __forceinline__ void step()
    {
        if ((pos & 15) == 0) {
            if ((pos & 31) == 0) word = p[min(pos >> 5, last_word)];
            cw = (pos & 16) ? (u32)word : (u32)(word >> 32);
        }
        const u32 b = __builtin_amdgcn_ubfe(cw, (u32)(30 - 2 * (pos & 15)), 2u);
        ++pos;
        fhi = __builtin_amdgcn_alignbit(fhi, flo, 30u) & (M ? ((1u << (2 * (M ? M : 17) - 32)) - 1u) : himask);
        flo = (flo << 2) | b;
        rlo = __builtin_amdgcn_alignbit(rhi, rlo, 2u);
        rhi = (rhi >> 2) | ((b ^ 3u) << (M ? (u32)(2 * (M ? M : 17) - 34) : rsh));
        st = (((u64)rhi << 32) | rlo) < (((u64)fhi << 32) | flo);
        clo = st ? rlo : flo;
        chi = st ? rhi : fhi;
    }
    __device__ __forceinline__ u32 hash() const { return order_hash32<M == 0>(((u64)chi << 32) | clo); }
    __device__ __forceinline__ u32 strand() const { return st ? 1u : 0u; }
};
#define RUN_W(e) ((u32)(e) >> 7)
#define RUN_DELTA(e) (((u32)(e) >> 1) & 63u)
#define RUN_STRAND(e) ((u32)(e)&1u)
#define OCC_MAKE(slot, e, wend) (((u32)(slot) << 29) | (RUN_STRAND(e) << 23) | (RUN_DELTA(e) << 17) | ((u32)(wend) << 8) | RUN_W(e))
#define OCC_SLOT(d) ((u32)(d) >> 29)
#define OCC_STRAND(d) (((u32)(d) >> 23) & 1u)
#define OCC_DELTA(d) (((u32)(d) >> 17) & 63u)
#define OCC_END(d) (((u32)(d) >> 8) & 0x1FFu)
#define OCC_FIRST(d) ((u32)(d)&0xFFu)

template <bool COUNT, int NF, int NL, int NFMAX = NF, bool LONGK = false>
__global__ void __launch_bounds__(256) index_runs_kernel(DiscoView v, u32 *__restrict__ bkt, ulonglong2 *__restrict__ rec, u32 *__restrict__ okey, u64 lo, u64 hi,
                                                         u32 *__restrict__ runs, u32 *__restrict__ ocnt, u32 *__restrict__ oslot, u64 *__restrict__ oitem, u32 oidbits,
                                                         u32 oshift, u32 osub,
                                                         const u64 *__restrict__ list = nullptr)
{
    static_assert(NF == 0 || NF == NFMAX, "a specialised instantiation holds exactly its window");
    constexpr int CAP = 32 * NL;
    __shared__ u16 s_runs[256 * CAP];
    __shared__ u32 s_x[3 * 256];
    const u32 tid = threadIdx.x;
    for (u32 x = tid; x < 256u * CAP / 2u; x += 256u) ((u32 *)s_runs)[x] = 0xFFFFFFFFu;
    __syncthreads();
    const u64 i = lo + (u64)blockIdx.x * 256u + tid;
    const u64 lw = (list && i < hi) ? list[i] : 0ull;
    const u64 rid = list ? ORDER_ID(lw) : i;
    const bool other_class = i < hi && v.full && v.len[rid] > DISCO_SHORT_MAX;
    if (other_class) s_runs[tid * CAP] = 0xFFFEu;
    const bool mine = i < hi && !other_class;
    const int L = mine ? (list ? ORDER_LEN(lw) : (int)v.len[rid]) : 0;
    int npos_lo = mine ? L - v.ks : 0x7FFFFFFF;
    for (int o = 32; o; o >>= 1) npos_lo = min(npos_lo, __shfl_xor(npos_lo, o));
    npos_lo = __builtin_amdgcn_readfirstlane(npos_lo);
    if (mine) {
        const u64 *__restrict__ p = v.reads + rid * v.S;
        const int k = v.ks;
        const int m = NF ? RUNS_M : v.m;
        const int nf = NF ? NF : k - m + 1;
        const int nmm = L - m + 1;
        const int npos = nmm - nf;
        MmerRoll<NF ? RUNS_M : 0> roll(p, v.S, m);
        u32 best = 0xFFFFFFFFu;
        for (int q = 0; q < m - 1; ++q) roll.step();
        u32 s1[NFMAX], s2[NFMAX];
#pragma clang loop unroll(full)
        for (int t = 0; t < NFMAX; ++t) s1[t] = s2[t] = 0xFFFFFFFFu;
        u16 *my = s_runs + tid * CAP;
        u32 cnt = 0, lastm = 0xFFFFFFFFu, tie = 0;
        u32 P1 = 0, P2 = 0;
        u32 sk = 0xFFFFFFFFu;
        u32 *sx = s_x + tid;
        auto window = [&](auto inner, int w, u32 m1, u32 m2, int base, int tw) __attribute__((always_inline)) {
            if (decltype(inner)::value || w <= npos) {
                if (!decltype(inner)::value && w == npos) {
                    sx[0] = m1;
                    sx[256] = m2;
                    sx[512] = (u32)base;
                } else {
                    tie |= (m1 ^ m2) ^ 0xFEu;
                    if (((m1 ^ lastm) >> 1) != 0u) {
                        lastm = m1;
                        my[cnt < (u32)CAP ? cnt : (u32)CAP - 1u] = (u16)((m1 & 0xFFu) + (((u32)w << 7) - 2u * (u32)tw));
                        sk = min(sk, (m1 & ~0x1FFu) | cnt);
                        ++cnt;
                    }
                }
            }
        };
        const int nblk = npos / nf + 2;
        int q = 0;
        auto block = [&](auto inner, int b) __attribute__((always_inline)) {
            const int base = (b - 1) * nf;
            lastm -= (u32)nf << 1;
            if (b >= 1) window(inner, base, s1[0], s2[0], base, 0);
            if (b == 1) {
                P1 = s1[0];
                P2 = s2[0];
            }
            u32 p1 = 0xFFFFFFFFu, p2 = 0xFFFFFFFFu;
            u32 hc[NFMAX];
#pragma clang loop unroll(full)
            for (int t = 0; t < NFMAX; ++t) {
                if (NF != 0 || t < nf) {
                    roll.step();
                    const u32 h = roll.hash();
                    best = min(best, decltype(inner)::value || q < nmm ? h : 0xFFFFFFFFu);
                    const u32 o = (h & ~0x1FFu) | roll.strand();
                    ++q;
                    hc[t] = o;
                    p1 = min(p1, o | ((u32)(nf + t) << 1));
                    p2 = min(p2, o | ((u32)(127 - (nf + t)) << 1));
                    if (t + 1 < nf && b >= 1) window(inner, base + t + 1, min(s1[t + 1 < NFMAX ? t + 1 : 0], p1), min(s2[t + 1 < NFMAX ? t + 1 : 0], p2), base, t + 1);
                }
            }
            u32 a1 = 0xFFFFFFFFu, a2 = 0xFFFFFFFFu;
#pragma clang loop unroll(full)
            for (int t = NFMAX - 1; t >= 0; --t) {
                if (NF == 0 && t >= nf) continue;
                a1 = min(a1, hc[t] | ((u32)t << 1));
                a2 = min(a2, hc[t] | ((u32)(127 - t) << 1));
                s1[t] = a1;
                s2[t] = a2;
            }
        };
        int b = 0;
        for (const int inner_end = npos_lo / nf; b <= inner_end; ++b) block(FlagConst<true>(), b);
        for (; b < nblk; ++b) block(FlagConst<false>(), b);
        if (okey) okey[i] = best;
        if (oitem) {
            u32 sub = 0;
            if (osub) {
                const u32 e = my[min(sk & 0x1FFu, (u32)CAP - 1u)];
                const u32 xm = sx[0];
                sub = ORDER_SUBKEY(min((sk & ~0x1FFu) | ((RUN_W(e) + RUN_DELTA(e)) << 1) | RUN_STRAND(e), (xm & ~0x1FFu) | ((xm & 0xFFu) + (sx[512] << 1))), nmm, osub);
            }
            oitem[i - lo] = ORDER_ITEM(best, oshift, rid, L, oidbits) | ((u64)sub << (32u + oshift - ORDER_SUB_BITS(osub)));
        }
        else if (ocnt) oslot[i - lo] = atomicAdd(&ocnt[ORDER_BUCKET(best, oshift)], 1u);
        if ((tie & ~1u) != 0 || cnt > (u32)CAP) my[0] = 0xFFFEu;
        auto resolve = [&](u32 k1, u32 k2, int wbase, int j0, u32 &t, u32 &rev) {
            const int ffirst = wbase + (int)((k1 >> 1) & 0x7Fu) - j0, flast = wbase + 127 - (int)((k2 >> 1) & 0x7Fu) - j0;
            int fsel = ffirst;
            if (ffirst == flast)
                rev = k1 & 1u;
            else {
                rev = kmer_is_rev<false, LONGK>(p, v.S, j0, k);
                fsel = rev ? flast : ffirst;
            }
            t = rev ? (u32)(nf - 1 - fsel) : (u32)fsel;
            return mmer_key(p, v.S, j0 + fsel, m);
        };
        u32 tp, rp, ts, rs;
        const u64 kp = resolve(P1, P2, 0, 0, tp, rp);
        const u64 ks = resolve(sx[0], sx[256], (int)sx[512], npos, ts, rs);
        const u64 bp = kp >> v.bshift, bs = ks >> v.bshift;
        const u32 sp = COUNT ? atomicAdd(&bkt[bp], 1u) : 0u;
        const u32 ss = COUNT ? atomicAdd(&bkt[bs], 1u) : 0u;
        rec[2 * (i - lo)] = make_ulonglong2((bp << 32) | sp, PAY_MAKE(kp, rid, tp, rp, 0, L));
        rec[2 * (i - lo) + 1] = make_ulonglong2((bs << 32) | ss, PAY_MAKE(ks, rid, ts, rs, 1, L));
    }
    __syncthreads();
#if defined(INDEX_EXP_NORUNS)
    if (tid != 9999u) return;
#endif
    const u64 r0 = (u64)blockIdx.x * 256u;
    const u64 nr = (hi - lo) - r0 < 256u ? (hi - lo) - r0 : 256u;
    u32 *__restrict__ dst = runs + r0 * (CAP / 2);
    for (u32 x = tid; x < (u32)nr * (CAP / 2); x += 256u) dst[x] = ((const u32 *)s_runs)[x];
}

__global__ void index_fill_kernel(u64 n2, const ulonglong2 *__restrict__ rec, const u32 *__restrict__ bkt, u64 *__restrict__ ent)
{
    u64 i = (u64)blockIdx.x * blockDim.x + threadIdx.x;
    for (; i < n2; i += (u64)gridDim.x * blockDim.x) {
        const ulonglong2 r = rec[i];
        ent[(u64)bkt[r.x >> 32] + (u32)r.x] = r.y;
    }
}

__global__ void index_fill_ordered_kernel(u64 nq, const u64 *__restrict__ order, const ulonglong2 *__restrict__ rec, const u32 *__restrict__ bkt, u64 *__restrict__ ent)
{
    u64 i = (u64)blockIdx.x * blockDim.x + threadIdx.x;
    for (; i < nq; i += (u64)gridDim.x * blockDim.x) {
        const u64 id = ORDER_ID(order[i]);
        const ulonglong2 r0 = rec[2 * id], r1 = rec[2 * id + 1];
        ent[(u64)bkt[r0.x >> 32] + (u32)r0.x] = r0.y;
        ent[(u64)bkt[r1.x >> 32] + (u32)r1.x] = r1.y;
    }
}

#define BINX_SPAN_BITS 14
#define BINX_MAX_BITS 8
#define BINX_TILE 2048u
#define BINX_BLOCK 256u
#define BINX_BUILD_BLOCK 1024u

__device__ __forceinline__ u32 binx_block_scan1024(u32 x, u32 *s_w, u32 *total)
{
    u32 incl = x;
    for (int o = 1; o < 64; o <<= 1) {
        const u32 y = __shfl_up(incl, o);
        if ((int)(threadIdx.x & 63) >= o) incl += y;
    }
    __syncthreads();
    if ((threadIdx.x & 63) == 63) s_w[threadIdx.x >> 6] = incl;
    __syncthreads();
    u32 off = 0, sum = 0;
    for (u32 w = 0; w < 16u; w++) {
        const u32 t = s_w[w];
        off += w < (threadIdx.x >> 6) ? t : 0u;
        sum += t;
    }
    *total = sum;
    return off + incl - x;
}

__global__ void __launch_bounds__(1024) binx_segs_kernel(const u32 *__restrict__ prev_scan, const u32 *__restrict__ ptb, u32 pseg, u32 pnb, u32 total, u32 *__restrict__ seg,
                                                         u32 *__restrict__ tb)
{
    __shared__ u32 s_w[16];
    const u32 nseg = prev_scan ? pseg * pnb : 1u;
    for (u32 x = threadIdx.x; x < nseg; x += 1024u) {
        u32 st = 0;
        if (prev_scan) {
            const u32 s = x / pnb, d = x % pnb;
            const u32 t0 = ptb[s], nt = ptb[s + 1] - t0;
            st = prev_scan[(u64)pnb * t0 + (u64)d * nt];
        }
        seg[x] = st;
    }
    if (threadIdx.x == 0) seg[nseg] = total;
    if (!tb) return;
    __syncthreads();
    u32 carry = 0;
    for (u32 base = 0; base < nseg; base += 1024u) {
        const u32 x = base + threadIdx.x;
        const u32 nt = x < nseg ? (seg[x + 1] - seg[x] + BINX_TILE - 1u) / BINX_TILE : 0u;
        u32 sum;
        const u32 ex = binx_block_scan1024(nt, s_w, &sum);
        if (x < nseg) tb[x] = carry + ex;
        carry += sum;
    }
    if (threadIdx.x == 0) tb[nseg] = carry;
}

__device__ __forceinline__ bool binx_tile(const u32 *__restrict__ seg, const u32 *__restrict__ tb, u32 nseg, u32 &t0, u32 &nt, u32 &ti, u32 &lo, u32 &hi)
{
    const u32 t = blockIdx.x;
    if (t >= tb[nseg]) return false;
    u32 a = 0, b = nseg;
    while (b - a > 1u) {
        const u32 mid = (a + b) >> 1;
        if (tb[mid] <= t) a = mid;
        else b = mid;
    }
    t0 = tb[a];
    nt = tb[a + 1] - t0;
    ti = t - t0;
    const u32 end = seg[a + 1];
    lo = seg[a] + ti * BINX_TILE;
    hi = end - lo > BINX_TILE ? lo + BINX_TILE : end;
    return true;
}

__device__ __forceinline__ u64 binx_key(const ulonglong2 &r) { return r.x; }
__device__ __forceinline__ u64 binx_key(u64 r) { return r; }
#define BINX_DIGIT(key, shift, nb) ((u32)((key) >> (shift)) & ((nb)-1u))

template <typename R>
__global__ void __launch_bounds__(BINX_BLOCK) binx_hist_kernel(const R *__restrict__ rec, const u32 *__restrict__ seg, const u32 *__restrict__ tb, u32 nseg, u32 shift, u32 nb,
                                                               u32 *__restrict__ hist)
{
    __shared__ u32 s_h[1u << BINX_MAX_BITS];
    u32 t0, nt, ti, lo, hi;
    if (!binx_tile(seg, tb, nseg, t0, nt, ti, lo, hi)) return;
    s_h[threadIdx.x] = 0;
    __syncthreads();
    for (u32 i = lo + threadIdx.x; i < hi; i += BINX_BLOCK) atomicAdd(&s_h[BINX_DIGIT(binx_key(rec[i]), shift, nb)], 1u);
    __syncthreads();
    if (threadIdx.x < nb) hist[(u64)nb * t0 + (u64)threadIdx.x * nt + ti] = s_h[threadIdx.x];
}

template <typename R>
__global__ void __launch_bounds__(BINX_BLOCK) binx_scatter_kernel(const R *__restrict__ src, R *__restrict__ dst, const u32 *__restrict__ seg, const u32 *__restrict__ tb,
                                                                  u32 nseg, u32 shift, u32 nb, const u32 *__restrict__ scan)
{
    static_assert(BINX_BLOCK == (1u << BINX_MAX_BITS) && BINX_TILE % BINX_BLOCK == 0, "a thread per bin; whole rounds per tile");
    constexpr u32 PER = BINX_TILE / BINX_BLOCK;
    __shared__ R s_rec[BINX_TILE];
    __shared__ u32 s_cnt[BINX_BLOCK], s_base[BINX_BLOCK], s_w[BINX_BLOCK / 64u];
    const u32 tid = threadIdx.x;
    u32 t0, nt, ti, lo, hi;
    if (!binx_tile(seg, tb, nseg, t0, nt, ti, lo, hi)) return;
    s_cnt[tid] = 0;
    __syncthreads();
    R r[PER];
    u32 rank[PER];
#pragma unroll
    for (u32 j = 0; j < PER; j++) {
        const u32 i = lo + j * BINX_BLOCK + tid;
        if (i < hi) {
            r[j] = src[i];
            rank[j] = atomicAdd(&s_cnt[BINX_DIGIT(binx_key(r[j]), shift, nb)], 1u);
        }
    }
    __syncthreads();
    const u32 cnt = s_cnt[tid];
    u32 incl = cnt;
    for (int o = 1; o < 64; o <<= 1) {
        const u32 y = __shfl_up(incl, o);
        if ((int)(tid & 63u) >= o) incl += y;
    }
    if ((tid & 63u) == 63u) s_w[tid >> 6] = incl;
    __syncthreads();
    u32 start = incl - cnt;
    for (u32 w = 0; w < (tid >> 6); w++) start += s_w[w];
    __syncthreads();
    s_cnt[tid] = start;
    if (tid < nb) s_base[tid] = scan[(u64)nb * t0 + (u64)tid * nt + ti] - start;
    __syncthreads();
#pragma unroll
    for (u32 j = 0; j < PER; j++) {
        const u32 i = lo + j * BINX_BLOCK + tid;
        if (i < hi) s_rec[s_cnt[BINX_DIGIT(binx_key(r[j]), shift, nb)] + rank[j]] = r[j];
    }
    __syncthreads();
    for (u32 j = tid; j < hi - lo; j += BINX_BLOCK) {
        const R x = s_rec[j];
        dst[s_base[BINX_DIGIT(binx_key(x), shift, nb)] + j] = x;
    }
}

__device__ __forceinline__ u64 binx_payload(const ulonglong2 &r, u32, u32) { return r.y; }
__device__ __forceinline__ u64 binx_payload(u64 r, u32 kshift, u32 idbits) { return ORDER_MAKE(r & ((1ull << idbits) - 1ull), (r << (64u - kshift)) >> (64u - kshift + idbits)); }
template <typename R>
__global__ void __launch_bounds__(BINX_BUILD_BLOCK) binx_build_kernel(const R *__restrict__ rec, const u32 *__restrict__ part, u32 span, u32 kshift, u32 idbits, u32 total, u64 T,
                                                                      u32 *__restrict__ bkt, u64 *__restrict__ ent)
{
    constexpr bool TABLE = sizeof(R) == sizeof(ulonglong2);
    __shared__ __attribute__((aligned(16))) u32 s_c[1u << BINX_SPAN_BITS];
    __shared__ u32 s_w[16];
    const u32 tid = threadIdx.x, p = blockIdx.x;
    const u32 nbk = 1u << span, mask = nbk - 1u;
    const u32 beg = part[p], end = part[p + 1];
    for (u32 x = tid; x < nbk / 4u; x += BINX_BUILD_BLOCK) ((uint4 *)s_c)[x] = make_uint4(0u, 0u, 0u, 0u);
    __syncthreads();
    for (u32 i = beg + tid; i < end; i += BINX_BUILD_BLOCK) atomicAdd(&s_c[(u32)(binx_key(rec[i]) >> kshift) & mask], 1u);
    __syncthreads();
    u32 carry = beg;
    if constexpr (!TABLE) {
        const u32 per4 = nbk / BINX_BUILD_BLOCK / 4u;
        uint4 *own = (uint4 *)(s_c + tid * per4 * 4u);
        u32 sum = 0;
        for (u32 j = 0; j < per4; j++) {
            const uint4 x = own[j];
            sum += x.x + x.y + x.z + x.w;
        }
        u32 all;
        u32 run = carry + binx_block_scan1024(sum, s_w, &all);
        for (u32 j = 0; j < per4; j++) {
            const uint4 x = own[j];
            uint4 y;
            y.x = run;
            y.y = y.x + x.x;
            y.z = y.y + x.y;
            y.w = y.z + x.z;
            run = y.w + x.w;
            own[j] = y;
        }
    } else
    for (u32 base = 0; base < nbk; base += BINX_BUILD_BLOCK) {
        const u32 x = s_c[base + tid];
        u32 sum;
        const u32 ex = binx_block_scan1024(x, s_w, &sum);
        s_c[base + tid] = carry + ex;
        if (TABLE) bkt[(u64)p * nbk + base + tid] = carry + ex;
        carry += sum;
    }
    if (TABLE && (u64)(p + 1u) * nbk == T && tid == 0) bkt[T] = total;
    __syncthreads();
    for (u32 i = beg + tid; i < end; i += BINX_BUILD_BLOCK) {
        const R x = rec[i];
        ent[atomicAdd(&s_c[(u32)(binx_key(x) >> kshift) & mask], 1u)] = binx_payload(x, kshift, idbits);
    }
}

template <typename InT>
__global__ void __launch_bounds__(SCAN_BLOCK) scan_tile_sums_kernel(const InT *__restrict__ in, u64 n, u64 *__restrict__ tile_sums)
{
    __shared__ u64 s_part[SCAN_BLOCK / DISCO_WAVE];
    u64 base = (u64)blockIdx.x * SCAN_TILE;
    u64 sum = 0;
    for (int i = 0; i < SCAN_ITEMS; i++) {
        u64 idx = base + (u64)i * SCAN_BLOCK + threadIdx.x;
        if (idx < n) sum += (u64)in[idx];
    }
    for (int o = 32; o > 0; o >>= 1) sum += __shfl_down(sum, o);
    if ((threadIdx.x & 63) == 0) s_part[threadIdx.x >> 6] = sum;
    __syncthreads();
    if (threadIdx.x == 0) {
        u64 t = 0;
        for (int w = 0; w < SCAN_BLOCK / DISCO_WAVE; w++) t += s_part[w];
        tile_sums[blockIdx.x] = t;
    }
}

__global__ void __launch_bounds__(1024) scan_sums_kernel(u64 *__restrict__ tile_sums, u64 nt, u64 *__restrict__ total)
{
    __shared__ u64 s_w[16];
    __shared__ u64 s_carry;
    if (threadIdx.x == 0) s_carry = 0;
    __syncthreads();
    for (u64 base = 0; base < nt; base += 1024) {
        u64 idx = base + threadIdx.x;
        u64 x = idx < nt ? tile_sums[idx] : 0;
        u64 incl = x;
        for (int o = 1; o < 64; o <<= 1) {
            u64 y = __shfl_up(incl, o);
            if ((int)(threadIdx.x & 63) >= o) incl += y;
        }
        if ((threadIdx.x & 63) == 63) s_w[threadIdx.x >> 6] = incl;
        __syncthreads();
        u64 woff = 0;
        for (int w = 0; w < (int)(threadIdx.x >> 6); w++) woff += s_w[w];
        u64 carry = s_carry;
        if (idx < nt) tile_sums[idx] = carry + woff + incl - x;
        __syncthreads();
        if (threadIdx.x == 1023) s_carry = carry + woff + incl;
        __syncthreads();
    }
    if (threadIdx.x == 0) *total = s_carry;
}

template <typename InT, typename OutT>
__global__ void __launch_bounds__(SCAN_BLOCK) scan_apply_kernel(const InT *in, u64 n, const u64 *__restrict__ tile_sums, OutT *out)
{
    __shared__ u64 s_w[SCAN_BLOCK / DISCO_WAVE];
    u64 base = (u64)blockIdx.x * SCAN_TILE + (u64)threadIdx.x * SCAN_ITEMS;
    u64 vals[SCAN_ITEMS];
    u64 sum = 0;
#pragma unroll
    for (int i = 0; i < SCAN_ITEMS; i++) {
        u64 idx = base + i;
        vals[i] = idx < n ? (u64)in[idx] : 0;
        sum += vals[i];
    }
    u64 incl = sum;
    for (int o = 1; o < 64; o <<= 1) {
        u64 y = __shfl_up(incl, o);
        if ((int)(threadIdx.x & 63) >= o) incl += y;
    }
    if ((threadIdx.x & 63) == 63) s_w[threadIdx.x >> 6] = incl;
    __syncthreads();
    u64 off = tile_sums[blockIdx.x] + incl - sum;
    for (int w = 0; w < (int)(threadIdx.x >> 6); w++) off += s_w[w];
#pragma unroll
    for (int i = 0; i < SCAN_ITEMS; i++) {
        u64 idx = base + i;
        if (idx < n) out[idx] = (OutT)off;
        off += vals[i];
    }
}

template <typename OutT>
__global__ void scan_write_total_kernel(const u64 *total, OutT *out_n) { *out_n = (OutT)*total; }

struct ProbeRare {
    u64 *bump;
    u64 hits_cap;
    u64 *big_list;
    u32 *big_cnt;
    u32 *n_big;
    u32 big_cap;
    u32 slow_cap;
    u64 *ctr;
    u64 *slow_list;
    u32 *n_slow;
};
struct ProbeArgs {
    DiscoView v;
    u64 *hits;
    u64 *row_start;
    u32 *row_cnt;
    ulonglong2 *meta_ord;
    const ProbeRare *rare;
    const u64 *order;
};

#ifndef PROBE_WAVES_PER_SIMD
#define PROBE_WAVES_PER_SIMD 8
#endif
template <int PMODE, bool LDSROW, bool ROW17, bool LONGK = false, bool LONGCLASS = false>
__global__ void __launch_bounds__(64, (LONGK || LONGCLASS) ? PROBE_WAVES_PER_SIMD - 2 : (ROW17 ? PROBE_WAVES_PER_SIMD - 1 : PROBE_WAVES_PER_SIMD)) probe_kernel(ProbeArgs a)
{
    static_assert(!LONGCLASS || (PMODE != 0 && !LDSROW), "the long class is only ever met in the lists");
    constexpr bool BIG = PMODE == 1, LISTED = PMODE != 0;
    __shared__ u32 s_k1[PROBE_SEGP + 32];
    __shared__ u32 s_k2[PROBE_SEGP + 32];
    __shared__ u8 s_strand[PROBE_SEGP];
    __shared__ u32 s_first[PROBE_SEGP];
    __shared__ u16 s_wp[PROBE_SEGW];
    __shared__ u16 s_lead[PROBE_SEGW];
    __shared__ u32 s_occ_fp[64];
    __shared__ u32 s_occ_start[64];
    __shared__ u32 s_occ_excl[64];
    __shared__ u16 s_occ_prel[64];
    __shared__ u8 s_mark[64];
    __shared__ u64 s_a[PROBE_ACAP + 2];
    const u32 lane = threadIdx.x;
    const int S = a.v.S, k = a.v.ks;
    const int m = a.v.m, nf = k - m + 1;
    const int dl = LONGK ? a.v.k - k : 0;
    u64 chunk_base = 0;
    u32 chunk_used = PROBE_CHUNK;
    u32 my_maxrow = 0;
    const u64 n_items = BIG ? (u64)min(*a.rare->n_big, a.rare->big_cap) : (PMODE == 2 ? (u64)min(*a.rare->n_slow, a.rare->slow_cap) : (a.v.q_hi - a.v.q_lo));

    u64 pre_w = 0;
    int pre_len = 0;
    u64 cbeg = 0, cend = 0;
    u64 ord_chunk = 0;
    auto rid = [&](u64 it) { return readlane_u64(ord_chunk, (u32)(it - cbeg)); };
    while (wq_grab(a.v.wq, n_items, cbeg, cend)) {
    if (!LISTED) {
        const u64 i = min(cbeg + lane, cend - 1);
        ord_chunk = a.order ? a.order[i] : ORDER_MAKE(a.v.q_lo + i, a.v.len[a.v.q_lo + i]);
    }
    if (!LISTED && LDSROW) {
        const u64 o0 = rid(cbeg);
        const u64 A0 = ORDER_ID(o0);
        pre_len = ORDER_LEN(o0);
        if ((int)lane < S) pre_w = a.v.reads[A0 * S + lane];
    }
    for (u64 it = cbeg; it < cend; it++) {
        const u64 bl = BIG ? a.rare->big_list[it] : (PMODE == 2 ? a.rare->slow_list[it] : 0ull);
        const u64 oe = LISTED ? 0ull : rid(it);
// ... 3725 lines not shown
```

Measured before the change: 11.76 billion overlaps/s.

## Store binned index records as split key/payload planes instead of 16-byte records

The binned index path now writes each record as a 32-bit bucket key plane plus a 64-bit payload plane instead of interleaved 16-byte records with a 64-bit key. The radix partition and build kernels read and move 12 bytes per record rather than 16, so the histogram passes only stream the 4-byte key plane. The build kernel loops are unrolled, and full tiles take a branch-free load path. The scratch buffer shrinks to 1.5n, and templating over record form adds code complexity.

```diff
diff --git a/disco_amd/csrc/disco_hip.hip b/disco_amd/csrc/disco_hip.hip
--- a/disco_amd/csrc/disco_hip.hip
+++ b/disco_amd/csrc/disco_hip.hip
@@ -972,69 +972,111 @@
     return DISCO_OK;
 }
 
-typedef void (*IndexRunsFn)(DiscoView, u32 *, ulonglong2 *, u32 *, u64, u64, u32 *, u32 *, u32 *, u64 *, u32, u32, u32, const u64 *);
-typedef void (*IndexCountFn)(DiscoView, u32 *, ulonglong2 *, u32 *, u64, u64, u32 *, u32 *, u64 *, u32, u32, const u64 *);
+typedef void (*IndexRunsFn)(DiscoView, u32 *, ulonglong2 *, u32 *, u64 *, u32 *, u64, u64, u32 *, u32 *, u32 *, u64 *, u32, u32, u32, const u64 *);
+typedef void (*IndexCountFn)(DiscoView, u32 *, ulonglong2 *, u32 *, u64 *, u32 *, u64, u64, u32 *, u32 *, u64 *, u32, u32, const u64 *);
 struct IndexCountKernel {
     IndexRunsFn runs = nullptr;
     IndexCountFn plain = nullptr;
 };
-template <bool COUNT, int NF, int NFMAX, bool LONGK>
+template <int OUT, int NF, int NFMAX, bool LONGK>
 static IndexCountKernel index_runs_pick(int lpr)
 {
     IndexCountKernel k;
-    k.runs = lpr == 16 ? index_runs_kernel<COUNT, NF, 1, NFMAX, LONGK> : index_runs_kernel<COUNT, NF, 2, NFMAX, LONGK>;
+    k.runs = lpr == 16 ? index_runs_kernel<OUT, NF, 1, NFMAX, LONGK> : index_runs_kernel<OUT, NF, 2, NFMAX, LONGK>;
     return k;
 }
-template <bool COUNT>
+template <int OUT>
 static IndexCountKernel index_count_pick(int nf, int m, int lpr, bool longk, bool long_class)
 {
     if (long_class || !lpr) {
         IndexCountKernel k;
-        if (long_class) k.plain = longk ? index_count_kernel<COUNT, true, true> : index_count_kernel<COUNT, false, true>;
-        else k.plain = longk ? index_count_kernel<COUNT, true> : index_count_kernel<COUNT>;
+        if (long_class) k.plain = longk ? index_count_kernel<OUT, true, true> : index_count_kernel<OUT, false, true>;
+        else k.plain = longk ? index_count_kernel<OUT, true> : index_count_kernel<OUT>;
         return k;
     }
     if (runs_nf_built(nf, m)) switch (nf) {
-        case 7: return index_runs_pick<COUNT, 7, 7, false>(lpr);
-        case 12: return index_runs_pick<COUNT, 12, 12, false>(lpr);
-        case 17: return index_runs_pick<COUNT, 17, 17, false>(lpr);
-        case 22: return index_runs_pick<COUNT, 22, 22, false>(lpr);
-        default: return index_runs_pick<COUNT, 27, 27, false>(lpr);
-        }
-    if (longk) return nf <= 48 ? index_runs_pick<COUNT, 0, 48, true>(lpr) : index_runs_pick<COUNT, 0, 64, true>(lpr);
-    if (nf <= 8) return index_runs_pick<COUNT, 0, 8, false>(lpr);
-    if (nf <= 12) return index_runs_pick<COUNT, 0, 12, false>(lpr);
-    if (nf <= 16) return index_runs_pick<COUNT, 0, 16, false>(lpr);
-    if (nf <= 24) return index_runs_pick<COUNT, 0, 24, false>(lpr);
-    if (nf <= 32) return index_runs_pick<COUNT, 0, 32, false>(lpr);
-    if (nf <= 48) return index_runs_pick<COUNT, 0, 48, false>(lpr);
-    return index_runs_pick<COUNT, 0, 64, false>(lpr);
-}
-static IndexCountKernel index_count_pick(bool count, int nf, int m, int lpr, bool longk, bool long_class)
-{
-    return count ? index_count_pick<true>(nf, m, lpr, longk, long_class) : index_count_pick<false>(nf, m, lpr, longk, long_class);
-}
-
-static int index_count_chunk(disco_ctx *c, const DiscoView &v, const IndexCountPlan &pl, bool count, ulonglong2 *rec_base, u64 a, u64 b)
+        case 7: return index_runs_pick<OUT, 7, 7, false>(lpr);
+        case 12: return index_runs_pick<OUT, 12, 12, false>(lpr);
+        case 17: return index_runs_pick<OUT, 17, 17, false>(lpr);
+        case 22: return index_runs_pick<OUT, 22, 22, false>(lpr);
+        default: return index_runs_pick<OUT, 27, 27, false>(lpr);
+        }
+    if (longk) return nf <= 48 ? index_runs_pick<OUT, 0, 48, true>(lpr) : index_runs_pick<OUT, 0, 64, true>(lpr);
+    if (nf <= 8) return index_runs_pick<OUT, 0, 8, false>(lpr);
+    if (nf <= 12) return index_runs_pick<OUT, 0, 12, false>(lpr);
+    if (nf <= 16) return index_runs_pick<OUT, 0, 16, false>(lpr);
+    if (nf <= 24) return index_runs_pick<OUT, 0, 24, false>(lpr);
+    if (nf <= 32) return index_runs_pick<OUT, 0, 32, false>(lpr);
+    if (nf <= 48) return index_runs_pick<OUT, 0, 48, false>(lpr);
+    return index_runs_pick<OUT, 0, 64, false>(lpr);
+}
+static IndexCountKernel index_count_pick(int out, int nf, int m, int lpr, bool longk, bool long_class)
+{
+    switch (out) {
+    case INDEX_COUNTED: return index_count_pick<INDEX_COUNTED>(nf, m, lpr, longk, long_class);
+    case INDEX_RECORDS: return index_count_pick<INDEX_RECORDS>(nf, m, lpr, longk, long_class);
+    default: return index_count_pick<INDEX_PLANES>(nf, m, lpr, longk, long_class);
+    }
+}
+
+struct IndexRecOut {
+    int form = INDEX_COUNTED;
+    ulonglong2 *rec = nullptr;
+    u32 *key = nullptr;
+    u64 *pay = nullptr;
+    IndexRecOut from_read(ptrdiff_t i) const
+    {
+        IndexRecOut o = *this;
+        if (o.rec) o.rec += 2 * i;
+        if (o.key) o.key += 2 * i, o.pay += 2 * i;
+        return o;
+    }
+};
+template <typename R>
+struct BinxSide {
+    typename BinxForm<R>::A *a = nullptr;
+    typename BinxForm<R>::B *b = nullptr;
+};
+static BinxSide<BinxKV> index_planes(ulonglong2 *side, u64 n)
+{
+    BinxSide<BinxKV> s;
+    s.b = (u64 *)side;
+    s.a = (u32 *)(s.b + 2 * n);
+    return s;
+}
+static IndexRecOut index_rec_out(disco_ctx *c)
+{
+    IndexRecOut o;
+    if (c->binned_index) {
+        const BinxSide<BinxKV> s = index_planes(c->d_rec.p, c->n);
+        o.form = INDEX_PLANES;
+        o.key = s.a;
+        o.pay = s.b;
+    } else
+        o.rec = c->d_rec.p;
+    return o;
+}
+
+static int index_count_chunk(disco_ctx *c, const DiscoView &v, const IndexCountPlan &pl, const IndexRecOut &out, u64 a, u64 b)
 {
     if (b <= a) return DISCO_OK;
     const dim3 grid((unsigned)((b - a + 255) / 256));
-    ulonglong2 *rec = rec_base + 2 * (a - pl.lo);
+    const IndexRecOut o = out.from_read((ptrdiff_t)(a - pl.lo));
     u32 *oslot = pl.oslot ? pl.oslot + (a - pl.lo) : nullptr;
     u64 *oitem = pl.oitem ? pl.oitem + (a - pl.lo) : nullptr;
     u32 *okey = pl.list ? nullptr : c->d_okey.p;
-    const IndexCountKernel k = index_count_pick(count, pl.nf, v.m, pl.lpr, c->ks > 64, false);
-    if (k.runs) hipLaunchKernelGGL(k.runs, grid, dim3(256), 0, c->stream, v, c->d_bkt, rec, okey, a, b, c->d_runs + (a - pl.lo) * (u64)pl.lpr, pl.ocnt, oslot, oitem, pl.oidbits, pl.oshift, pl.osub, pl.list);
-    else hipLaunchKernelGGL(k.plain, grid, dim3(256), 0, c->stream, v, c->d_bkt, rec, okey, a, b, pl.ocnt, oslot, oitem, pl.oidbits, pl.oshift, pl.list);
+    const IndexCountKernel k = index_count_pick(o.form, pl.nf, v.m, pl.lpr, c->ks > 64, false);
+    if (k.runs) hipLaunchKernelGGL(k.runs, grid, dim3(256), 0, c->stream, v, c->d_bkt, o.rec, o.key, o.pay, okey, a, b, c->d_runs + (a - pl.lo) * (u64)pl.lpr, pl.ocnt, oslot, oitem, pl.oidbits, pl.oshift, pl.osub, pl.list);
+    else hipLaunchKernelGGL(k.plain, grid, dim3(256), 0, c->stream, v, c->d_bkt, o.rec, o.key, o.pay, okey, a, b, pl.ocnt, oslot, oitem, pl.oidbits, pl.oshift, pl.list);
     HIPCHK(c, hipGetLastError());
     return DISCO_OK;
 }
 
-static int index_count_long(disco_ctx *c, const DiscoView &v, const IndexCountPlan &pl, bool count, ulonglong2 *rec, u32 *oslot, u64 x_lo, u64 x_hi)
+static int index_count_long(disco_ctx *c, const DiscoView &v, const IndexCountPlan &pl, const IndexRecOut &out, u32 *oslot, u64 x_lo, u64 x_hi)
 {
     const dim3 g((unsigned)((x_hi - x_lo + 255) / 256));
-    hipLaunchKernelGGL(index_count_pick(count, 0, v.m, 0, c->ks > 64, true).plain, g, dim3(256), 0, c->stream, v, c->d_bkt, rec, c->d_okey, x_lo, x_hi, pl.ocnt, oslot, (u64 *)nullptr, 0u, pl.oshift,
-                       (const u64 *)nullptr);
+    hipLaunchKernelGGL(index_count_pick(out.form, 0, v.m, 0, c->ks > 64, true).plain, g, dim3(256), 0, c->stream, v, c->d_bkt, out.rec, out.key, out.pay, c->d_okey, x_lo, x_hi, pl.ocnt, oslot,
+                       (u64 *)nullptr, 0u, pl.oshift, (const u64 *)nullptr);
     HIPCHK(c, hipGetLastError());
     return DISCO_OK;
 }
@@ -1042,7 +1084,7 @@
 static bool binned_index_wanted(disco_ctx *c, int logT)
 {
     if (getenv("DISCO_NO_BINNED_INDEX") || 2 * c->n >= 0xFFFF0000ull) return false;
-    if (logT > BINX_SPAN_BITS && ensure(c, c->d_rec2, 2 * c->n) != DISCO_OK) {
+    if (logT > BINX_SPAN_BITS && ensure(c, c->d_rec2, (3 * c->n + 1) / 2) != DISCO_OK) {
         (void)hipGetLastError();
         c->err.clear();
         return false;
@@ -1093,8 +1135,10 @@
 }
 
 template <typename R>
-static int binx_partition(disco_ctx *c, const char *what, int bits, u32 kshift, u32 total, R *src, R *dst, const R **out, const u32 **part)
-{
+static int binx_partition(disco_ctx *c, const char *what, int bits, u32 kshift, u32 total, BinxSide<R> src, BinxSide<R> dst, BinxSide<R> *out, const u32 **part)
+{
+    typedef typename BinxForm<R>::A A;
+    typedef typename BinxForm<R>::B B;
     const BinxPlan bp = binx_plan(bits);
     const u32 n_part = 1u << (bits - bp.span);
     const u32 tiles = (total + BINX_TILE - 1u) / BINX_TILE;
@@ -1113,9 +1157,10 @@
         const u64 hlen = (u64)grid * nb + 1;
         hipLaunchKernelGGL(binx_segs_kernel, dim3(1), dim3(1024), 0, c->stream, l ? (const u32 *)hist : (const u32 *)nullptr, (const u32 *)tb[cur ^ 1], pseg, pnb, total, seg[cur], tb[cur]);
         HIPCHK(c, hipMemsetAsync(hist, 0, hlen * sizeof(u32), c->stream));
-        hipLaunchKernelGGL(binx_hist_kernel<R>, dim3(grid), dim3(BINX_BLOCK), 0, c->stream, (const R *)src, (const u32 *)seg[cur], (const u32 *)tb[cur], nseg, shift, nb, hist);
+        hipLaunchKernelGGL(binx_hist_kernel<R>, dim3(grid), dim3(BINX_BLOCK), 0, c->stream, (const A *)src.a, (const u32 *)seg[cur], (const u32 *)tb[cur], nseg, shift, nb, hist);
         CHK((scan_exclusive<u32, u32>(c, hist, hlen, hist, false, nullptr)));
-        hipLaunchKernelGGL(binx_scatter_kernel<R>, dim3(grid), dim3(BINX_BLOCK), 0, c->stream, (const R *)src, dst, (const u32 *)seg[cur], (const u32 *)tb[cur], nseg, shift, nb, (const u32 *)hist);
+        hipLaunchKernelGGL(binx_scatter_kernel<R>, dim3(grid), dim3(BINX_BLOCK), 0, c->stream, (const A *)src.a, (const B *)src.b, dst.a, dst.b, (const u32 *)seg[cur], (const u32 *)tb[cur], nseg, shift, nb,
+                           (const u32 *)hist);
         HIPCHK(c, hipGetLastError());
         std::swap(src, dst);
         pseg = nseg;
@@ -1135,11 +1180,12 @@
 {
     const int logT = 64 - c->bshift;
     const u32 total = (u32)(2 * c->n);
-    const ulonglong2 *rec;
+    BinxSide<BinxKV> rec;
     const u32 *part;
-    CHK(binx_partition(c, "index build", logT, 32u, total, c->d_rec.p, c->d_rec2.p, &rec, &part));
+    CHK(binx_partition<BinxKV>(c, "index build", logT, 0u, total, index_planes(c->d_rec.p, c->n), index_planes(c->d_rec2.p, c->n), &rec, &part));
     const int span = std::min(logT, BINX_SPAN_BITS);
-    hipLaunchKernelGGL(binx_build_kernel<ulonglong2>, dim3(1u << (logT - span)), dim3(BINX_BUILD_BLOCK), 0, c->stream, rec, part, (u32)span, 32u, 0u, total, c->T, c->d_bkt.p, c->d_ent.p);
+    hipLaunchKernelGGL(binx_build_kernel<BinxKV>, dim3(1u << (logT - span)), dim3(BINX_BUILD_BLOCK), 0, c->stream, (const u32 *)rec.a, (const u64 *)rec.b, part, (u32)span, 0u, 0u, total, c->T,
+                       c->d_bkt.p, c->d_ent.p);
     HIPCHK(c, hipGetLastError());
     return DISCO_OK;
 }
@@ -1148,12 +1194,13 @@
 {
     const int bits = c->order_counted_bits + c->order_sub_bits;
     const u32 total = (u32)c->n, kshift = 64u - (u32)bits;
-    u64 *items = (u64 *)c->d_rec2.p;
-    const u64 *rec;
+    BinxSide<u64> items, other, rec;
+    items.a = (u64 *)c->d_rec2.p;
+    other.a = items.a + c->n;
     const u32 *part;
-    CHK(binx_partition(c, "grouping", bits, kshift, total, items, items + c->n, &rec, &part));
+    CHK(binx_partition<u64>(c, "grouping", bits, kshift, total, items, other, &rec, &part));
     const int span = std::min(bits, BINX_SPAN_BITS);
-    hipLaunchKernelGGL(binx_build_kernel<u64>, dim3(1u << (bits - span)), dim3(BINX_BUILD_BLOCK), 0, c->stream, rec, part, (u32)span, kshift, (u32)c->order_id_bits, total, (u64)0,
+    hipLaunchKernelGGL(binx_build_kernel<u64>, dim3(1u << (bits - span)), dim3(BINX_BUILD_BLOCK), 0, c->stream, (const u64 *)rec.a, (const u64 *)nullptr, part, (u32)span, kshift, (u32)c->order_id_bits, total, (u64)0,
                        (u32 *)nullptr, c->d_order_own.p);
     HIPCHK(c, hipGetLastError());
     return DISCO_OK;
@@ -1801,7 +1848,7 @@
                 HIPCHK(c, hipEventRecord(c->ev_copied[b], c->copy_stream));
                 HIPCHK(c, hipStreamWaitEvent(c->stream, c->ev_copied[b], 0));
             }
-            if (eager) CHK(index_count_chunk(c, v, pl, !c->binned_index, c->d_rec, lo, hi));
+            if (eager) CHK(index_count_chunk(c, v, pl, index_rec_out(c), lo, hi));
         }
         HIPCHK(c, hipGetLastError());
         t_issued = lapms();
@@ -2718,8 +2765,8 @@
         const DiscoView v = view(c);
         IndexCountPlan pl;
         CHK(index_count_plan(c, v, 0, c->n, &pl));
-        CHK(index_count_chunk(c, v, pl, !c->binned_index, c->d_rec, 0, c->n));
-        if (c->two_class) CHK(index_count_long(c, v, pl, !c->binned_index, c->d_rec, pl.oslot, 0, c->n_long));
+        CHK(index_count_chunk(c, v, pl, index_rec_out(c), 0, c->n));
+        if (c->two_class) CHK(index_count_long(c, v, pl, index_rec_out(c), pl.oslot, 0, c->n_long));
     }
     const bool binned = c->binned_index;
     if (!binned) CHK((scan_exclusive<u32, u32>(c, c->d_bkt, c->T + 1, c->d_bkt, false, nullptr)));
@@ -5430,21 +5477,24 @@
     ph_begin(c, DISCO_PH_INDEX);
     DiscoView v = view(c);
     IndexCountPlan pl;
+    IndexRecOut rec_out;
+    rec_out.form = INDEX_RECORDS;
+    rec_out.rec = c->d_rec.p;
     if (c->loci) {
         CHK(index_count_plan(c, v, 0, c->n_own, &pl, c->d_order_own));
-        CHK(index_count_chunk(c, v, pl, false, c->d_rec, 0, c->n_own));
+        CHK(index_count_chunk(c, v, pl, rec_out, 0, c->n_own));
     } else {
         CHK(index_count_plan(c, v, c->q_lo, c->q_hi, &pl));
-        CHK(index_count_chunk(c, v, pl, false, c->d_rec, c->q_lo, c->q_hi));
+        CHK(index_count_chunk(c, v, pl, rec_out, c->q_lo, c->q_hi));
         if (c->two_class && nloc) {
             u32 xb[2] = {0, (u32)c->n_long};
             HIPCHK(c, hipMemcpyAsync(&xb[0], c->d_ovf + c->q_lo, sizeof(u32), hipMemcpyDeviceToHost, c->stream));
             if (c->q_hi < c->n) HIPCHK(c, hipMemcpyAsync(&xb[1], c->d_ovf + c->q_hi, sizeof(u32), hipMemcpyDeviceToHost, c->stream));
             HIPCHK(c, hipStreamSynchronize(c->stream));
             if (xb[1] > xb[0]) {
-                ulonglong2 *rec_by_id = c->d_rec - 2 * (ptrdiff_t)c->q_lo;
+                const IndexRecOut rec_by_id = rec_out.from_read(-(ptrdiff_t)c->q_lo);
                 u32 *oslot_by_id = pl.oslot ? pl.oslot - (ptrdiff_t)c->q_lo : nullptr;
-                CHK(index_count_long(c, v, pl, false, rec_by_id, oslot_by_id, xb[0], xb[1]));
+                CHK(index_count_long(c, v, pl, rec_by_id, oslot_by_id, xb[0], xb[1]));
             }
         }
     }
diff --git a/disco_amd/csrc/disco_kernels.h b/disco_amd/csrc/disco_kernels.h
--- a/disco_amd/csrc/disco_kernels.h
+++ b/disco_amd/csrc/disco_kernels.h
@@ -241,8 +241,25 @@
     }
 }
 
-template <bool COUNT, bool LONGK = false, bool LONGCLASS = false>
-__global__ void __launch_bounds__(256) index_count_kernel(DiscoView v, u32 *__restrict__ bkt, ulonglong2 *__restrict__ rec, u32 *__restrict__ okey, u64 lo, u64 hi,
+enum IndexOut { INDEX_COUNTED = 0, INDEX_RECORDS = 1, INDEX_PLANES = 2 };
+template <int OUT>
+__device__ __forceinline__ void index_put_pair(u32 *__restrict__ bkt, ulonglong2 *__restrict__ rec, u32 *__restrict__ pkey, u64 *__restrict__ ppay, u64 j, u64 bp, u64 pp, u64 bs,
+                                               u64 ps)
+{
+    if constexpr (OUT == INDEX_PLANES) {
+        ((uint2 *)pkey)[j] = make_uint2((u32)bp, (u32)bs);
+        ((ulonglong2 *)ppay)[j] = make_ulonglong2(pp, ps);
+    } else {
+        const u32 sp = OUT == INDEX_COUNTED ? atomicAdd(&bkt[bp], 1u) : 0u;
+        const u32 ss = OUT == INDEX_COUNTED ? atomicAdd(&bkt[bs], 1u) : 0u;
+        rec[2 * j] = make_ulonglong2((bp << 32) | sp, pp);
+        rec[2 * j + 1] = make_ulonglong2((bs << 32) | ss, ps);
+    }
+}
+
+template <int OUT, bool LONGK = false, bool LONGCLASS = false>
+__global__ void __launch_bounds__(256) index_count_kernel(DiscoView v, u32 *__restrict__ bkt, ulonglong2 *__restrict__ rec, u32 *__restrict__ pkey, u64 *__restrict__ ppay,
+                                                          u32 *__restrict__ okey, u64 lo, u64 hi,
                                                           u32 *__restrict__ ocnt, u32 *__restrict__ oslot, u64 *__restrict__ oitem, u32 oidbits, u32 oshift,
                                                           const u64 *__restrict__ list = nullptr)
 {
@@ -315,10 +332,7 @@
     const u64 kp = resolve(k1p, k2p, 0, tp, rp);
     const u64 ks = resolve(k1s, k2s, sfx0, ts, rs);
     const u64 bp = kp >> v.bshift, bs = ks >> v.bshift;
-    const u32 sp = COUNT ? atomicAdd(&bkt[bp], 1u) : 0u;
-    const u32 ss = COUNT ? atomicAdd(&bkt[bs], 1u) : 0u;
-    rec[2 * (i - lo)] = make_ulonglong2((bp << 32) | sp, PAY_MAKE(kp, rid, tp, rp, 0, L));
-    rec[2 * (i - lo) + 1] = make_ulonglong2((bs << 32) | ss, PAY_MAKE(ks, LONGCLASS ? v.n + x : rid, ts, rs, 1, L));
+    index_put_pair<OUT>(bkt, rec, pkey, ppay, i - lo, bp, PAY_MAKE(kp, rid, tp, rp, 0, L), bs, PAY_MAKE(ks, LONGCLASS ? v.n + x : rid, ts, rs, 1, L));
 }
 
 #define RUNS_M 23
@@ -368,8 +382,9 @@
 #define OCC_END(d) (((u32)(d) >> 8) & 0x1FFu)
 #define OCC_FIRST(d) ((u32)(d)&0xFFu)
 
-template <bool COUNT, int NF, int NL, int NFMAX = NF, bool LONGK = false>
-__global__ void __launch_bounds__(256) index_runs_kernel(DiscoView v, u32 *__restrict__ bkt, ulonglong2 *__restrict__ rec, u32 *__restrict__ okey, u64 lo, u64 hi,
+template <int OUT, int NF, int NL, int NFMAX = NF, bool LONGK = false>
+__global__ void __launch_bounds__(256) index_runs_kernel(DiscoView v, u32 *__restrict__ bkt, ulonglong2 *__restrict__ rec, u32 *__restrict__ pkey, u64 *__restrict__ ppay,
+                                                         u32 *__restrict__ okey, u64 lo, u64 hi,
                                                          u32 *__restrict__ runs, u32 *__restrict__ ocnt, u32 *__restrict__ oslot, u64 *__restrict__ oitem, u32 oidbits,
                                                          u32 oshift, u32 osub,
                                                          const u64 *__restrict__ list = nullptr)
@@ -493,10 +508,7 @@
         const u64 kp = resolve(P1, P2, 0, 0, tp, rp);
         const u64 ks = resolve(sx[0], sx[256], (int)sx[512], npos, ts, rs);
         const u64 bp = kp >> v.bshift, bs = ks >> v.bshift;
-        const u32 sp = COUNT ? atomicAdd(&bkt[bp], 1u) : 0u;
-        const u32 ss = COUNT ? atomicAdd(&bkt[bs], 1u) : 0u;
-        rec[2 * (i - lo)] = make_ulonglong2((bp << 32) | sp, PAY_MAKE(kp, rid, tp, rp, 0, L));
-        rec[2 * (i - lo) + 1] = make_ulonglong2((bs << 32) | ss, PAY_MAKE(ks, rid, ts, rs, 1, L));
+        index_put_pair<OUT>(bkt, rec, pkey, ppay, i - lo, bp, PAY_MAKE(kp, rid, tp, rp, 0, L), bs, PAY_MAKE(ks, rid, ts, rs, 1, L));
     }
     __syncthreads();
 #if defined(INDEX_EXP_NORUNS)
@@ -533,6 +545,7 @@
 #define BINX_TILE 2048u
 #define BINX_BLOCK 256u
 #define BINX_BUILD_BLOCK 1024u
+#define BINX_BUILD_UNROLL 4u
 
 __device__ __forceinline__ u32 binx_block_scan1024(u32 x, u32 *s_w, u32 *total)
 {
@@ -602,31 +615,86 @@
     return true;
 }
 
-__device__ __forceinline__ u64 binx_key(const ulonglong2 &r) { return r.x; }
-__device__ __forceinline__ u64 binx_key(u64 r) { return r; }
 #define BINX_DIGIT(key, shift, nb) ((u32)((key) >> (shift)) & ((nb)-1u))
 
 template <typename R>
-__global__ void __launch_bounds__(BINX_BLOCK) binx_hist_kernel(const R *__restrict__ rec, const u32 *__restrict__ seg, const u32 *__restrict__ tb, u32 nseg, u32 shift, u32 nb,
-                                                               u32 *__restrict__ hist)
-{
+struct BinxForm;
+template <>
+struct BinxForm<u64> {
+    typedef u64 A;
+    typedef u64 B;
+    static constexpr bool TABLE = false;
+    struct Stage {
+        u64 r[BINX_TILE];
+    };
+    static __device__ __forceinline__ u64 key_at(const A *__restrict__ a, u32 i) { return a[i]; }
+    static __device__ __forceinline__ u64 key(const u64 &r) { return r; }
+    static __device__ __forceinline__ u64 load(const A *__restrict__ a, const B *__restrict__, u32 i) { return a[i]; }
+    static __device__ __forceinline__ void store(A *__restrict__ a, B *__restrict__, u32 j, const u64 &r) { a[j] = r; }
+    static __device__ __forceinline__ void stage(Stage &s, u32 j, const u64 &r) { s.r[j] = r; }
+    static __device__ __forceinline__ u64 staged(const Stage &s, u32 j) { return s.r[j]; }
+};
+struct BinxKV {
+    u64 pay;
+    u32 key;
+};
+template <>
+struct BinxForm<BinxKV> {
+    typedef u32 A;
+    typedef u64 B;
+    static constexpr bool TABLE = true;
+    struct Stage {
+        u64 pay[BINX_TILE];
+        u32 key[BINX_TILE];
+    };
+    static __device__ __forceinline__ u32 key_at(const A *__restrict__ a, u32 i) { return a[i]; }
+    static __device__ __forceinline__ u32 key(const BinxKV &r) { return r.key; }
+    static __device__ __forceinline__ BinxKV load(const A *__restrict__ a, const B *__restrict__ b, u32 i) { return BinxKV{b[i], a[i]}; }
+    static __device__ __forceinline__ void store(A *__restrict__ a, B *__restrict__ b, u32 j, const BinxKV &r)
+    {
+        a[j] = r.key;
+        b[j] = r.pay;
+    }
+    static __device__ __forceinline__ void stage(Stage &s, u32 j, const BinxKV &r)
+    {
+        s.key[j] = r.key;
+        s.pay[j] = r.pay;
+    }
+    static __device__ __forceinline__ BinxKV staged(const Stage &s, u32 j) { return BinxKV{s.pay[j], s.key[j]}; }
+};
+
+template <typename R>
+__global__ void __launch_bounds__(BINX_BLOCK) binx_hist_kernel(const typename BinxForm<R>::A *__restrict__ rec, const u32 *__restrict__ seg, const u32 *__restrict__ tb, u32 nseg,
+                                                               u32 shift, u32 nb, u32 *__restrict__ hist)
+{
+    typedef BinxForm<R> F;
     __shared__ u32 s_h[1u << BINX_MAX_BITS];
     u32 t0, nt, ti, lo, hi;
     if (!binx_tile(seg, tb, nseg, t0, nt, ti, lo, hi)) return;
     s_h[threadIdx.x] = 0;
     __syncthreads();
-    for (u32 i = lo + threadIdx.x; i < hi; i += BINX_BLOCK) atomicAdd(&s_h[BINX_DIGIT(binx_key(rec[i]), shift, nb)], 1u);
+    if (hi - lo == BINX_TILE) {
+        constexpr u32 PER = BINX_TILE / BINX_BLOCK;
+        decltype(F::key_at(rec, 0u)) k[PER];
+#pragma unroll
+        for (u32 j = 0; j < PER; j++) k[j] = F::key_at(rec, lo + j * BINX_BLOCK + threadIdx.x);
+#pragma unroll
+        for (u32 j = 0; j < PER; j++) atomicAdd(&s_h[BINX_DIGIT(k[j], shift, nb)], 1u);
+    } else
+        for (u32 i = lo + threadIdx.x; i < hi; i += BINX_BLOCK) atomicAdd(&s_h[BINX_DIGIT(F::key_at(rec, i), shift, nb)], 1u);
     __syncthreads();
     if (threadIdx.x < nb) hist[(u64)nb * t0 + (u64)threadIdx.x * nt + ti] = s_h[threadIdx.x];
 }
 
 template <typename R>
-__global__ void __launch_bounds__(BINX_BLOCK) binx_scatter_kernel(const R *__restrict__ src, R *__restrict__ dst, const u32 *__restrict__ seg, const u32 *__restrict__ tb,
-                                                                  u32 nseg, u32 shift, u32 nb, const u32 *__restrict__ scan)
+__global__ void __launch_bounds__(BINX_BLOCK) binx_scatter_kernel(const typename BinxForm<R>::A *__restrict__ src, const typename BinxForm<R>::B *__restrict__ srcb,
+                                                                  typename BinxForm<R>::A *__restrict__ dst, typename BinxForm<R>::B *__restrict__ dstb, const u32 *__restrict__ seg,
+                                                                  const u32 *__restrict__ tb, u32 nseg, u32 shift, u32 nb, const u32 *__restrict__ scan)
 {
     static_assert(BINX_BLOCK == (1u << BINX_MAX_BITS) && BINX_TILE % BINX_BLOCK == 0, "a thread per bin; whole rounds per tile");
+    typedef BinxForm<R> F;
     constexpr u32 PER = BINX_TILE / BINX_BLOCK;
-    __shared__ R s_rec[BINX_TILE];
+    __shared__ typename F::Stage s_rec;
     __shared__ u32 s_cnt[BINX_BLOCK], s_base[BINX_BLOCK], s_w[BINX_BLOCK / 64u];
     const u32 tid = threadIdx.x;
     u32 t0, nt, ti, lo, hi;
@@ -635,12 +703,19 @@
     __syncthreads();
     R r[PER];
     u32 rank[PER];
-#pragma unroll
-    for (u32 j = 0; j < PER; j++) {
-        const u32 i = lo + j * BINX_BLOCK + tid;
-        if (i < hi) {
-            r[j] = src[i];
-            rank[j] = atomicAdd(&s_cnt[BINX_DIGIT(binx_key(r[j]), shift, nb)], 1u);
+    if (hi - lo == BINX_TILE) {
+#pragma unroll
+        for (u32 j = 0; j < PER; j++) r[j] = F::load(src, srcb, lo + j * BINX_BLOCK + tid);
+#pragma unroll
+        for (u32 j = 0; j < PER; j++) rank[j] = atomicAdd(&s_cnt[BINX_DIGIT(F::key(r[j]), shift, nb)], 1u);
+    } else {
+#pragma unroll
+        for (u32 j = 0; j < PER; j++) {
+            const u32 i = lo + j * BINX_BLOCK + tid;
+            if (i < hi) {
+                r[j] = F::load(src, srcb, i);
+                rank[j] = atomicAdd(&s_cnt[BINX_DIGIT(F::key(r[j]), shift, nb)], 1u);
+            }
         }
     }
     __syncthreads();
@@ -661,22 +736,24 @@
 #pragma unroll
     for (u32 j = 0; j < PER; j++) {
         const u32 i = lo + j * BINX_BLOCK + tid;
-        if (i < hi) s_rec[s_cnt[BINX_DIGIT(binx_key(r[j]), shift, nb)] + rank[j]] = r[j];
+        if (i < hi) F::stage(s_rec, s_cnt[BINX_DIGIT(F::key(r[j]), shift, nb)] + rank[j], r[j]);
     }
     __syncthreads();
     for (u32 j = tid; j < hi - lo; j += BINX_BLOCK) {
-        const R x = s_rec[j];
-        dst[s_base[BINX_DIGIT(binx_key(x), shift, nb)] + j] = x;
-    }
-}
-
-__device__ __forceinline__ u64 binx_payload(const ulonglong2 &r, u32, u32) { return r.y; }
+        const R x = F::staged(s_rec, j);
+        F::store(dst, dstb, s_base[BINX_DIGIT(F::key(x), shift, nb)] + j, x);
+    }
+}
+
 __device__ __forceinline__ u64 binx_payload(u64 r, u32 kshift, u32 idbits) { return ORDER_MAKE(r & ((1ull << idbits) - 1ull), (r << (64u - kshift)) >> (64u - kshift + idbits)); }
+__device__ __forceinline__ u64 binx_payload(const BinxKV &r, u32, u32) { return r.pay; }
 template <typename R>
-__global__ void __launch_bounds__(BINX_BUILD_BLOCK) binx_build_kernel(const R *__restrict__ rec, const u32 *__restrict__ part, u32 span, u32 kshift, u32 idbits, u32 total, u64 T,
-                                                                      u32 *__restrict__ bkt, u64 *__restrict__ ent)
-{
-    constexpr bool TABLE = sizeof(R) == sizeof(ulonglong2);
+__global__ void __launch_bounds__(BINX_BUILD_BLOCK) binx_build_kernel(const typename BinxForm<R>::A *__restrict__ rec, const typename BinxForm<R>::B *__restrict__ recb,
+                                                                      const u32 *__restrict__ part, u32 span, u32 kshift, u32 idbits, u32 total, u64 T, u32 *__restrict__ bkt,
+                                                                      u64 *__restrict__ ent)
+{
+    typedef BinxForm<R> F;
+    constexpr bool TABLE = F::TABLE;
     __shared__ __attribute__((aligned(16))) u32 s_c[1u << BINX_SPAN_BITS];
     __shared__ u32 s_w[16];
     const u32 tid = threadIdx.x, p = blockIdx.x;
@@ -684,7 +761,15 @@
     const u32 beg = part[p], end = part[p + 1];
     for (u32 x = tid; x < nbk / 4u; x += BINX_BUILD_BLOCK) ((uint4 *)s_c)[x] = make_uint4(0u, 0u, 0u, 0u);
     __syncthreads();
-    for (u32 i = beg + tid; i < end; i += BINX_BUILD_BLOCK) atomicAdd(&s_c[(u32)(binx_key(rec[i]) >> kshift) & mask], 1u);
+    u32 i = beg + tid;
+    for (; i + (BINX_BUILD_UNROLL - 1u) * BINX_BUILD_BLOCK < end; i += BINX_BUILD_UNROLL * BINX_BUILD_BLOCK) {
+        decltype(F::key_at(rec, 0u)) k[BINX_BUILD_UNROLL];
+#pragma unroll
+        for (u32 u = 0; u < BINX_BUILD_UNROLL; u++) k[u] = F::key_at(rec, i + u * BINX_BUILD_BLOCK);
+#pragma unroll
+        for (u32 u = 0; u < BINX_BUILD_UNROLL; u++) atomicAdd(&s_c[(u32)(k[u] >> kshift) & mask], 1u);
+    }
+    for (; i < end; i += BINX_BUILD_BLOCK) atomicAdd(&s_c[(u32)(F::key_at(rec, i) >> kshift) & mask], 1u);
     __syncthreads();
     u32 carry = beg;
     if constexpr (!TABLE) {
@@ -718,9 +803,17 @@
     }
     if (TABLE && (u64)(p + 1u) * nbk == T && tid == 0) bkt[T] = total;
     __syncthreads();
-    for (u32 i = beg + tid; i < end; i += BINX_BUILD_BLOCK) {
-        const R x = rec[i];
-        ent[atomicAdd(&s_c[(u32)(binx_key(x) >> kshift) & mask], 1u)] = binx_payload(x, kshift, idbits);
+    i = beg + tid;
+    for (; i + (BINX_BUILD_UNROLL - 1u) * BINX_BUILD_BLOCK < end; i += BINX_BUILD_UNROLL * BINX_BUILD_BLOCK) {
+        R x[BINX_BUILD_UNROLL];
+#pragma unroll
+        for (u32 u = 0; u < BINX_BUILD_UNROLL; u++) x[u] = F::load(rec, recb, i + u * BINX_BUILD_BLOCK);
+#pragma unroll
+        for (u32 u = 0; u < BINX_BUILD_UNROLL; u++) ent[atomicAdd(&s_c[(u32)(F::key(x[u]) >> kshift) & mask], 1u)] = binx_payload(x[u], kshift, idbits);
+    }
+    for (; i < end; i += BINX_BUILD_BLOCK) {
+        const R x = F::load(rec, recb, i);
+        ent[atomicAdd(&s_c[(u32)(F::key(x) >> kshift) & mask], 1u)] = binx_payload(x, kshift, idbits);
     }
 }
 
```

After: 11.94 billion overlaps/s (median of 6 runs). 1.02x the previous value.
